# ducha-aiki/affnet

Measured on NVIDIA H100. Metric: Mpix/s end-to-end HesAffNet(+OriNet)+HardNet, higher is better.
Workload: dtype fp16 operands (fp16 residual planes: AffNet/OriNet weights+activations, HardNet layer 2-3 weights), fp32 accumulate; stencils fp32

## Files before the change

### affnet_b200/_lib.py

```python
import ctypes as C
import os
import subprocess

import torch

HERE = os.path.dirname(os.path.abspath(__file__))
LIB_PATH = os.environ.get("AFFNET_B200_LIB", os.path.join(HERE, "lib", "libaffnet_b200.so"))
AG_MAX_OCTAVES, AG_MAX_LEVELS = 16, 8
NET_AFFNET, NET_ORINET, NET_HARDNET = 0, 1, 2
ENGINE_SIMT, ENGINE_TC, ENGINE_TC_EXACT, ENGINE_TC_FAST, ENGINE_TC2, ENGINE_TC2_BF16 = 0, 1, 2, 3, 4, 5


class AffnetB200Error(RuntimeError):
    pass


class PyramidPlan(C.Structure):
    _fields_ = [
        ("B", C.c_int), ("H", C.c_int), ("W", C.c_int), ("n_octaves", C.c_int), ("n_levels", C.c_int),
        ("h", C.c_int * AG_MAX_OCTAVES), ("w", C.c_int * AG_MAX_OCTAVES),
        ("level_offset", (C.c_longlong * AG_MAX_LEVELS) * AG_MAX_OCTAVES),
        ("total_floats", C.c_longlong),
        ("sigma", (C.c_double * AG_MAX_LEVELS) * AG_MAX_OCTAVES),
        ("blur_sigma", (C.c_double * AG_MAX_LEVELS) * AG_MAX_OCTAVES),
        ("pix_dist", C.c_double * AG_MAX_OCTAVES),
    ]


class DetectWs(C.Structure):
    _fields_ = [
        ("B", C.c_int), ("cand_cap", C.c_int), ("n_level_slots", C.c_int),
        ("d_cand_val", C.c_void_p), ("d_cand_seq", C.c_void_p), ("d_cand_scyx", C.c_void_p), ("d_cand_aux", C.c_void_p),
        ("d_cand_count", C.c_void_p), ("d_level_pos", C.c_void_p), ("d_level_emit", C.c_void_p), ("d_variants", C.c_void_p),
        ("d_octave_maps", C.c_void_p),
    ]


class PipelineConfig(C.Structure):
    _fields_ = [
        ("B", C.c_int), ("H", C.c_int), ("W", C.c_int), ("num_features", C.c_int), ("nlevels", C.c_int),
        ("border", C.c_int), ("init_sigma", C.c_double), ("mrSize", C.c_double), ("do_ori", C.c_int),
        ("cand_cap", C.c_int),
    ]


SHAPE_NONE, SHAPE_AFFNET, SHAPE_BAUMBERG = 0, 1, 2
ORI_NONE, ORI_ORINET, ORI_HISTOGRAM = 0, 1, 2


class PipelineEstimators(C.Structure):
    _fields_ = [("shape", C.c_int), ("num_baum_iters", C.c_int), ("shape_ps", C.c_int), ("ori", C.c_int), ("ori_ps", C.c_int)]


DESC_HARDNET, DESC_SIFT = 0, 1


class PipelineDescriptor(C.Structure):
    _fields_ = [("kind", C.c_int), ("ps", C.c_int), ("clipval", C.c_float)]


vp, i32, f32, f64, sz = C.c_void_p, C.c_int, C.c_float, C.c_double, C.c_size_t
PROTOTYPES = {
    "ag_last_error": (C.c_char_p, []),
    "ag_abi_version": (i32, []),
    "ag_prof_begin": (i32, [vp]),
    "ag_prof_end": (i32, []),
    "ag_prof_get": (i32, [i32, C.POINTER(C.c_char_p), C.POINTER(f32)]),
    "ag_pyramid_plan": (i32, [i32, i32, i32, i32, f64, i32, C.POINTER(PyramidPlan)]),
    "ag_pyramid_build": (i32, [C.POINTER(PyramidPlan), vp, vp, vp]),
    "ag_gaussian_blur": (i32, [vp, vp, i32, i32, i32, f64, vp]),
    "ag_hessian_response": (i32, [vp, vp, i32, i32, i32, f64, f32, vp]),
    "ag_detect_ws_bytes": (sz, [C.POINTER(PyramidPlan), i32]),
    "ag_detect_ws_carve": (i32, [C.POINTER(PyramidPlan), i32, vp, C.POINTER(DetectWs)]),
    "ag_detect": (i32, [C.POINTER(PyramidPlan), vp, f32, i32, C.POINTER(DetectWs), vp]),
    "ag_detect_level_from_responses": (i32, [vp, vp, vp, i32, i32, C.POINTER(f64), i32, vp, vp, i32, C.POINTER(DetectWs), vp]),
    "ag_select_keypoints": (i32, [C.POINTER(PyramidPlan), C.POINTER(DetectWs), i32, f32, i32, vp, vp, vp, vp, vp, vp]),
    "ag_select_all_workspace_bytes": (sz, [C.POINTER(PyramidPlan), i32]),
    "ag_select_all_keypoints": (i32, [C.POINTER(PyramidPlan), C.POINTER(DetectWs), f32, i32, vp, sz, vp, vp, vp, vp, vp, vp]),
    "ag_extract_patches": (i32, [vp, i32, i32, i32, i32, vp, i32, i32, vp, vp]),
    "ag_extract_patches_pyr": (i32, [C.POINTER(PyramidPlan), vp, vp, vp, vp, vp, i32, i32, vp, vp]),
    "ag_pyramid_level_for_lafs": (i32, [C.POINTER(PyramidPlan), vp, i32, i32, vp, vp, vp]),
    "ag_net_create": (i32, [i32, vp, sz, C.POINTER(vp)]),
    "ag_net_destroy": (None, [vp]),
    "ag_net_blob_floats": (sz, [i32]),
    "ag_net_set_engine": (i32, [vp, i32]),
    "ag_net_get_engine": (i32, [vp]),
    "ag_net_workspace_bytes": (sz, [i32, i32]),
    "ag_mat2_compose": (i32, [vp, vp, vp, i32, vp]),
    "ag_lafs_left_multiply": (i32, [vp, vp, vp, i32, vp]),
    "ag_affnet_forward_raw": (i32, [vp, vp, i32, vp, vp, sz, vp]),
    "ag_orinet_forward_raw": (i32, [vp, vp, i32, vp, vp, sz, vp]),
    "ag_debug_pyramid_mode": (i32, [i32]),
    "ag_debug_tcx_layer": (i32, [vp, vp, i32, i32, vp, vp, sz, vp]),
    "ag_debug_libm": (i32, [vp, vp, i32, vp, vp, vp, vp]),
    "ag_debug_orientation_hist_pyr": (i32, [C.POINTER(PyramidPlan), vp, vp, vp, vp, vp, i32, i32, vp, vp, vp]),
    "ag_debug_baumberg_pyr": (i32, [C.POINTER(PyramidPlan), vp, vp, vp, vp, vp, i32, i32, i32, vp, vp, vp]),
    "ag_affnet_forward": (i32, [vp, vp, i32, vp, i32, vp, vp, sz, vp]),
    "ag_orinet_forward": (i32, [vp, vp, i32, vp, i32, vp, vp, vp, sz, vp]),
    "ag_hardnet_forward": (i32, [vp, vp, i32, vp, i32, vp, vp, sz, vp]),
    "ag_net_forward_pyr": (i32, [vp, C.POINTER(PyramidPlan), vp, vp, vp, vp, vp, i32, vp, vp, sz, vp]),
    "ag_affine_shape_filter": (i32, [vp, vp, vp, vp, vp, vp, i32, i32, i32, i32, vp, vp, vp, vp, vp, vp]),
    "ag_affine_shape_filter_all": (i32, [vp, vp, vp, vp, vp, vp, i32, i32, vp, vp, vp, vp, vp, vp]),
    "ag_lafs_apply_rotation": (i32, [vp, vp, i32, vp]),
    "ag_lafs_scale": (i32, [vp, vp, i32, f32, f32, f32, vp]),
    "ag_lafs_to_ell": (i32, [vp, i32, vp, vp]),
    "ag_circular_gauss_kernel": (i32, [i32, f64, vp]),
    "ag_orientation_hist": (i32, [vp, i32, i32, vp, vp, vp]),
    "ag_baumberg_shape": (i32, [vp, i32, i32, vp, vp, vp]),
    "ag_sift_windows": (i32, [i32, vp, vp, C.POINTER(i32), C.POINTER(i32)]),
    "ag_sift_describe": (i32, [vp, i32, i32, f32, vp, vp]),
    "ag_sift_describe_pyr": (i32, [C.POINTER(PyramidPlan), vp, vp, vp, vp, vp, i32, i32, f32, vp, vp]),
    "ag_distance_matrix": (i32, [vp, i32, vp, i32, i32, vp, vp]),
    "ag_match_snn_workspace_bytes": (sz, [i32, i32]),
    "ag_match_snn": (i32, [vp, i32, vp, i32, i32, f32, vp, sz, vp, vp, vp, vp, vp]),
    "ag_match_pairs_workspace_bytes": (sz, [i32, i32, i32, i32, i32]),
    "ag_match_pairs": (i32, [vp, vp, i32, i32, vp, vp, i32, i32, i32, vp, i32, f32, vp, sz, vp, vp, vp, vp, vp, vp, vp]),
    "ag_homography_ransac": (i32, [vp, i32, i32, vp, i32, i32, vp, i32, vp, vp, i32, f32, f32, i32, C.c_uint64, vp, vp, vp, vp, vp]),
    "ag_gt_correspondences_pairs": (i32, [vp, i32, i32, vp, i32, i32, vp, i32, vp, vp, i32, vp, f32, vp, vp, vp, vp, vp]),
    "ag_pipeline_create": (i32, [C.POINTER(PipelineConfig), vp, vp, vp, C.POINTER(vp)]),
    "ag_pipeline_create_ex": (i32, [C.POINTER(PipelineConfig), C.POINTER(PipelineEstimators), vp, vp, vp, C.POINTER(vp)]),
    "ag_pipeline_create_desc": (i32, [C.POINTER(PipelineConfig), C.POINTER(PipelineEstimators), C.POINTER(PipelineDescriptor), vp, vp, vp,
                                      C.POINTER(vp)]),
    "ag_pipeline_create_th": (i32, [C.POINTER(PipelineConfig), C.POINTER(PipelineEstimators), C.POINTER(PipelineDescriptor), f32, vp, vp, vp,
                                    C.POINTER(vp)]),
    "ag_pipeline_destroy": (None, [vp]),
    "ag_pipeline_workspace_bytes": (sz, [vp]),
    "ag_pipeline_plan": (C.POINTER(PyramidPlan), [vp]),
    "ag_pipeline_run": (i32, [vp, vp, vp, sz, vp, vp, vp, vp, vp]),
    "ag_pipeline_launch_count": (i32, [vp]),
}

_lib = None


def build(verbose=False):
    r = subprocess.run(["bash", os.path.join(HERE, "csrc", "build.sh")], capture_output=True, text=True)
    if r.returncode != 0:
        raise AffnetB200Error("building libaffnet_b200.so failed:\n" + r.stdout + r.stderr)
    if verbose:
        print(r.stdout.strip())
    return LIB_PATH


def lib():
    global _lib
    if _lib is None:
        if not os.path.isfile(LIB_PATH):
            raise AffnetB200Error("%s not found: run `python -c 'import __graft_entry__ as g; g.build()'` "
                                  "(there is no CPU fallback)" % LIB_PATH)
        L = C.CDLL(LIB_PATH)
        for name, (res, args) in PROTOTYPES.items():
            fn = getattr(L, name)
            fn.restype, fn.argtypes = res, args
        _lib = L
    return _lib


def check(rc):
    if rc != 0:
        raise AffnetB200Error("libaffnet_b200 error %d: %s" % (rc, lib().ag_last_error().decode()))


def stream_ptr():
    return C.c_void_p(torch.cuda.current_stream().cuda_stream)


def ptr(t):
    if t is None:
        return C.c_void_p(0)
    return C.c_void_p(t.data_ptr())


def require_cuda(t, name="tensor"):
    if not (isinstance(t, torch.Tensor) and t.is_cuda):
        raise AffnetB200Error("%s must be a CUDA tensor: affnet_b200 has no CPU path" % name)
    return t


def f32c(t, name="tensor"):
    require_cuda(t, name)
    if t.dtype != torch.float32:
        t = t.float()
    return t.contiguous()


def make_plan(B, H, W, nlevels=3, init_sigma=1.6, border=5):
    plan = PyramidPlan()
    check(lib().ag_pyramid_plan(B, H, W, nlevels, float(init_sigma), border, C.byref(plan)))
    return plan


def profile(fn):
    check(lib().ag_prof_begin(stream_ptr()))
    try:
        fn()
    finally:
        n = lib().ag_prof_end()
    if n < 0:
        check(n)
    out = []
    for i in range(n):
        name, ms = C.c_char_p(), C.c_float()
        check(lib().ag_prof_get(i, C.byref(name), C.byref(ms)))
        out.append((name.value.decode(), ms.value))
    return out
```

### affnet_b200/csrc/net_impl.cuh

```cuda
#pragma once
#include <cuda_fp16.h>

#include <vector>

#include "common.cuh"

#define AG_ENGINE_SIMT 0
#define AG_ENGINE_TC 1
#define AG_ENGINE_TC_EXACT 2
#define AG_ENGINE_TC2 4
#define AG_ENGINE_TC2_BF16 5
#define AG_ENGINE_TC_FAST 3

struct ag_net {
    int kind;
    int engine;
    float* d_w[6];
    float* d_b[6];
    float* d_w1;
    __half* d_wx[6];
    __half* d_all_x;
    __half* d_wx_bf[6];
    __half* d_headh_bf;
    __half* d_wh[6];
    __half* d_headh;
    float* d_head_w;
    float* d_head_b;
    float* d_head_bx;
    float w_inv_scale[6];
    float head_inv_scale;
    float* d_all;
    __half* d_all_h;
};

#include "tc_conv.cuh"

namespace ag {
size_t tc_act_bytes(int kind);
int tc_nsplit(int kind, int layer);
int tc_split_w(int kind);
tc::FirstSrc tc_src_patches(const float* patches);
tc::FirstSrc tc_src_pyramid(const ag_pyramid_plan_t* p, const float* pyr, const float* lafs, const int* oct, const int* lvl, int cap);
int tc_hardnet_forward(const ag_net* net, const tc::FirstSrc& src, int n, int group, const int* count, void* bufA, void* bufB, void* headbuf,
                       float* out, cudaStream_t st);
int tc_trunk_orinet(const ag_net* net, const tc::FirstSrc& src, int n, int group, const int* count, void* bufA, void* bufB, void* feat,
                    cudaStream_t st);
int tc_trunk_affnet(const ag_net* net, const tc::FirstSrc& src, int n, int group, const int* count, void* bufA, void* bufB, void* feat,
                    cudaStream_t st);
int tc_headx_forward(const ag_net* net, const void* feat, int n, int group, const int* count, float* out, float* angle, cudaStream_t st, float* raw = nullptr);
size_t tc_headx_bytes(int n);
void tcx_pack_layer(const float* wf, int ci, int co, int stride, int nsplit, int sw, float scale, std::vector<__half>& out, int bf16 = 0);
int tcx_nsplit(int kind, int layer);
int tcx_split_w(int kind, int layer);
int tcx_stride(int layer);
size_t tcx_act_bytes(int n);
int tcx_trunk_affori(const ag_net* net, const tc::FirstSrc& src, int n, int group, const int* count, void* bufA, void* bufB, void* feat,
                     cudaStream_t st, int upto);
int tcx_trunk_hardnet(const ag_net* net, const tc::FirstSrc& src, int n, int group, const int* count, void* bufA, void* bufB, void* headbuf,
                      cudaStream_t st, int upto, int bf16 = 0);
int tc_hardnet_head(const ag_net* net, const void* headbuf, int n, int group, const int* count, float* out, cudaStream_t st, int bf16 = 0);
}
```

### affnet_b200/csrc/nets_simt.cu

```cuda
#include <math.h>

#include <vector>

#include <cuda_bf16.h>

#include "net_impl.cuh"

namespace ag {

constexpr float BN_EPS = 1e-5f;
constexpr int CNT = 256;

struct LayerCfg {
    int cin, cout, stride, hin;
};
static const LayerCfg kAffCfg[6] = {{1, 16, 1, 32}, {16, 16, 1, 32}, {16, 32, 2, 32}, {32, 32, 1, 16}, {32, 64, 2, 16}, {64, 64, 1, 8}};
static const LayerCfg kHardCfg[6] = {{1, 32, 1, 32}, {32, 32, 1, 32}, {32, 64, 2, 32}, {64, 64, 1, 16}, {64, 128, 2, 16}, {128, 128, 1, 8}};

}

namespace ag {

template <int CIN, int COUT, int HIN, int STRIDE, int CT, int CK, bool NORM>
__global__ void __launch_bounds__(CNT) conv3x3_kernel(const float* __restrict__ in, float* __restrict__ out,
                                                       const float* __restrict__ wpk, const float* __restrict__ bias,
                                                       int group, const int* __restrict__ count) {
    constexpr int HOUT = HIN / STRIDE, NP = HOUT * HOUT, PPT = 4, PT = NP / PPT, CGN = CNT / PT, CPT = CT / CGN;
    constexpr int HP = HIN + 2, WP = HIN + 2;
    static_assert(PT * CGN == CNT && CPT * CGN == CT && CPT % 4 == 0, "bad tiling");
    static_assert(CIN % CK == 0, "bad cin chunk");
    extern __shared__ float smem[];
    float* s_in = smem;
    float* s_w = smem + CIN * HP * WP;
    __shared__ float s_red[CNT / 32][2];

    const int pi = blockIdx.x;
    if (count != nullptr && (pi % group) >= count[pi / group]) return;
    const int ct0 = blockIdx.y * CT;
    const float* src = in + (size_t)pi * CIN * HIN * HIN;

    float mean = 0.f, inv = 1.f;
    if (NORM) {
        float s = 0.f;
        for (int i = threadIdx.x; i < HIN * HIN; i += CNT) s += src[i];
        for (int o = 16; o > 0; o >>= 1) s += __shfl_xor_sync(0xffffffffu, s, o);
        if ((threadIdx.x & 31) == 0) s_red[threadIdx.x >> 5][0] = s;
        __syncthreads();
        s = 0.f;
        for (int i = 0; i < CNT / 32; i++) s += s_red[i][0];
        mean = s / (float)(HIN * HIN);
        float q = 0.f;
        for (int i = threadIdx.x; i < HIN * HIN; i += CNT) { const float d = src[i] - mean; q = fmaf(d, d, q); }
        for (int o = 16; o > 0; o >>= 1) q += __shfl_xor_sync(0xffffffffu, q, o);
        if ((threadIdx.x & 31) == 0) s_red[threadIdx.x >> 5][1] = q;
        __syncthreads();
        q = 0.f;
        for (int i = 0; i < CNT / 32; i++) q += s_red[i][1];
        inv = 1.f / (sqrtf(q / (float)(HIN * HIN - 1)) + 1e-7f);
    }
    for (int i = threadIdx.x; i < CIN * HP * WP; i += CNT) {
        const int c = i / (HP * WP), r = i - c * HP * WP, y = r / WP, x = r - y * WP;
        float v = 0.f;
        if (y >= 1 && y <= HIN && x >= 1 && x <= HIN) {
            v = src[(size_t)c * HIN * HIN + (y - 1) * HIN + (x - 1)];
            if (NORM) v = (v - mean) * inv;
        }
        s_in[i] = v;
    }

    const int pt = threadIdx.x % PT, cg = threadIdx.x / PT;
    int poff[PPT];
#pragma unroll
    for (int k = 0; k < PPT; k++) {
        const int p = pt + k * PT, y = p / HOUT, x = p - y * HOUT;
        poff[k] = (y * STRIDE) * WP + x * STRIDE;
    }
    float acc[PPT][CPT];
#pragma unroll
    for (int j = 0; j < CPT; j++) {
        const float bv = bias[ct0 + cg * CPT + j];
#pragma unroll
        for (int k = 0; k < PPT; k++) acc[k][j] = bv;
    }

    for (int c0 = 0; c0 < CIN; c0 += CK) {
        __syncthreads();
        for (int i = threadIdx.x; i < 9 * CK * CT; i += CNT) {
            const int tap = i / (CK * CT), r = i - tap * CK * CT, c = r / CT, co = r - c * CT;
            s_w[i] = __ldg(wpk + ((size_t)tap * CIN + c0 + c) * COUT + ct0 + co);
        }
        __syncthreads();
#pragma unroll 1
        for (int c = 0; c < CK; c++) {
            const float* ip = s_in + (c0 + c) * HP * WP;
#pragma unroll
            for (int tap = 0; tap < 9; tap++) {
                const int toff = (tap / 3) * WP + (tap % 3);
                float a[PPT];
#pragma unroll
                for (int k = 0; k < PPT; k++) a[k] = ip[poff[k] + toff];
                const float4* wp = reinterpret_cast<const float4*>(s_w + (tap * CK + c) * CT + cg * CPT);
#pragma unroll
                for (int j4 = 0; j4 < CPT / 4; j4++) {
                    const float4 wv = wp[j4];
#pragma unroll
                    for (int k = 0; k < PPT; k++) {
                        acc[k][j4 * 4 + 0] = fmaf(a[k], wv.x, acc[k][j4 * 4 + 0]);
                        acc[k][j4 * 4 + 1] = fmaf(a[k], wv.y, acc[k][j4 * 4 + 1]);
                        acc[k][j4 * 4 + 2] = fmaf(a[k], wv.z, acc[k][j4 * 4 + 2]);
                        acc[k][j4 * 4 + 3] = fmaf(a[k], wv.w, acc[k][j4 * 4 + 3]);
                    }
                }
            }
        }
    }
    float* dst = out + (size_t)pi * COUT * NP;
#pragma unroll
    for (int j = 0; j < CPT; j++)
#pragma unroll
        for (int k = 0; k < PPT; k++) dst[(size_t)(ct0 + cg * CPT + j) * NP + pt + k * PT] = fmaxf(acc[k][j], 0.f);
}

template <int CIN, int COUT, int HIN, int STRIDE, int CT, int CK, bool NORM>
static int launch_conv(const float* in, float* out, const float* w, const float* b, int n, int group, const int* count,
                       cudaStream_t st) {
    constexpr size_t smem = sizeof(float) * ((size_t)CIN * (HIN + 2) * (HIN + 2) + 9 * CK * CT);
    static SmemAttrOnce attr_once;
    auto kern = conv3x3_kernel<CIN, COUT, HIN, STRIDE, CT, CK, NORM>;
    {
        int rc = attr_once.ensure(kern, smem, "conv smem attr");
        if (rc != AG_OK) return rc;
    }
    kern<<<dim3(n, COUT / CT), CNT, smem, st>>>(in, out, w, b, group, count);
    AG_CHECK_LAUNCH("conv3x3_kernel");
    return AG_OK;
}

__device__ __forceinline__ float warp_sum(float v) {
    for (int o = 16; o > 0; o >>= 1) v += __shfl_xor_sync(0xffffffffu, v, o);
    return v;
}

__global__ void affnet_head_kernel(const float* __restrict__ feat, const float* __restrict__ w, const float* __restrict__ bias,
                                   float* __restrict__ out, int n, int group, const int* __restrict__ count) {
    const int pi = blockIdx.x * (blockDim.x >> 5) + (threadIdx.x >> 5), lane = threadIdx.x & 31;
    if (pi >= n) return;
    if (count != nullptr && (pi % group) >= count[pi / group]) return;
    const float* f = feat + (size_t)pi * 4096;
    float s0 = 0.f, s1 = 0.f, s2 = 0.f;
    for (int i = lane; i < 4096; i += 32) {
        const float v = f[i];
        s0 = fmaf(v, __ldg(w + i), s0); s1 = fmaf(v, __ldg(w + 4096 + i), s1); s2 = fmaf(v, __ldg(w + 8192 + i), s2);
    }
    s0 = warp_sum(s0); s1 = warp_sum(s1); s2 = warp_sum(s2);
    if (lane == 0) {
        const float a00 = 1.0f + tanhf(s0 + bias[0]), a10 = tanhf(s1 + bias[1]), a11 = 1.0f + tanhf(s2 + bias[2]);
        rectify_up_is_up(a00, 0.f, a10, a11, out + (size_t)pi * 4);
    }
}

constexpr int OH_P = 4, OH_W = 8, OH_KC = 256;
__global__ void __launch_bounds__(OH_W * 32) orinet_head_kernel(const float* __restrict__ feat, const float* __restrict__ weff, const float* __restrict__ bias,
                                                                 float* __restrict__ out, float* __restrict__ angle_out, int n, int group,
                                                                 const int* __restrict__ count) {
    __shared__ __align__(16) float s_w[OH_KC][20];
    const int warp = threadIdx.x >> 5, lane = threadIdx.x & 31;
    const int p0 = (blockIdx.x * OH_W + warp) * OH_P;
    float acc[OH_P][18];
#pragma unroll
    for (int q = 0; q < OH_P; q++)
#pragma unroll
        for (int o = 0; o < 18; o++) acc[q][o] = 0.f;
    const float* f[OH_P];
#pragma unroll
    for (int q = 0; q < OH_P; q++) f[q] = feat + (size_t)min(p0 + q, n - 1) * 4096;
    for (int k0 = 0; k0 < 4096; k0 += OH_KC) {
        __syncthreads();
        for (int i = threadIdx.x; i < OH_KC * 18; i += OH_W * 32) s_w[i / 18][i % 18] = __ldg(weff + (size_t)k0 * 18 + i);
        __syncthreads();
#pragma unroll 2
        for (int kk = lane; kk < OH_KC; kk += 32) {
            float v[OH_P];
#pragma unroll
            for (int q = 0; q < OH_P; q++) v[q] = f[q][k0 + kk];
            const float4* wr = reinterpret_cast<const float4*>(&s_w[kk][0]);
            const float4 w0 = wr[0], w1 = wr[1], w2 = wr[2], w3 = wr[3];
            const float2 w4 = *reinterpret_cast<const float2*>(&s_w[kk][16]);
            const float wv[18] = {w0.x, w0.y, w0.z, w0.w, w1.x, w1.y, w1.z, w1.w, w2.x, w2.y, w2.z, w2.w, w3.x, w3.y, w3.z, w3.w, w4.x, w4.y};
#pragma unroll
            for (int q = 0; q < OH_P; q++)
#pragma unroll
                for (int o = 0; o < 18; o++) acc[q][o] = fmaf(v[q], wv[o], acc[q][o]);
        }
    }
#pragma unroll
    for (int q = 0; q < OH_P; q++) {
        float m0 = 0.f, m1 = 0.f;
#pragma unroll
        for (int o = 0; o < 9; o++) {
            m0 += tanhf(warp_sum(acc[q][o]) + bias[0]);
            m1 += tanhf(warp_sum(acc[q][9 + o]) + bias[1]);
        }
        const int pi = p0 + q;
        if (lane != 0 || pi >= n) continue;
        if (count != nullptr && (pi % group) >= count[pi / group]) continue;
        m0 /= 9.0f; m1 /= 9.0f;
        const float ang = atan2f(m0 + 1e-8f, m1 + 1e-8f);
        if (angle_out) angle_out[pi] = ang;
        if (out) {
            const float c = cosf(ang), sn = sinf(ang);
            float* o = out + (size_t)pi * 4;
            o[0] = c; o[1] = sn; o[2] = -sn; o[3] = c;
        }
    }
}

constexpr int HH_P = 16;
__global__ void __launch_bounds__(256) hardnet_head_kernel(const float* __restrict__ feat, const float* __restrict__ w,
                                                            const float* __restrict__ bn, float* __restrict__ out, int n,
                                                            int group, const int* __restrict__ count) {
    __shared__ float s_a[HH_P][64 + 1];
    const int p0 = blockIdx.x * HH_P;
    const int co = threadIdx.x & 127, half = threadIdx.x >> 7;
    float acc[HH_P / 2];
#pragma unroll
    for (int k = 0; k < HH_P / 2; k++) acc[k] = 0.f;
    for (int k0 = 0; k0 < 8192; k0 += 64) {
        __syncthreads();
        for (int i = threadIdx.x; i < HH_P * 64; i += 256) {
            const int p = i >> 6, k = i & 63;
            s_a[p][k] = (p0 + p < n) ? feat[(size_t)(p0 + p) * 8192 + k0 + k] : 0.f;
        }
        __syncthreads();
#pragma unroll 8
        for (int k = 0; k < 64; k++) {
            const float wv = __ldg(w + (size_t)(k0 + k) * 128 + co);
#pragma unroll
            for (int q = 0; q < HH_P / 2; q++) acc[q] = fmaf(s_a[half * (HH_P / 2) + q][k], wv, acc[q]);
        }
    }
    const float sc = bn[co], sh = bn[128 + co];
    float v[HH_P / 2];
#pragma unroll
    for (int q = 0; q < HH_P / 2; q++) v[q] = fmaf(acc[q], sc, sh);
    __syncthreads();
    const int wih = (threadIdx.x >> 5) & 3;
#pragma unroll
    for (int q = 0; q < HH_P / 2; q++) {
        const float ss = warp_sum(v[q] * v[q]);
        if ((threadIdx.x & 31) == 0) s_a[half * (HH_P / 2) + q][wih] = ss;
    }
    __syncthreads();
#pragma unroll
    for (int q = 0; q < HH_P / 2; q++) {
        const int r = half * (HH_P / 2) + q, p = p0 + r;
        if (p >= n) continue;
        if (count != nullptr && (p % group) >= count[p / group]) continue;
        const float ss = (s_a[r][0] + s_a[r][1]) + (s_a[r][2] + s_a[r][3]);
        out[(size_t)p * 128 + co] = v[q] / sqrtf(ss + 1e-8f);
    }
}

static float pow2_scale(const float* w, size_t n) {
    float wmax = 0.f;
    for (size_t i = 0; i < n; i++) wmax = fmaxf(wmax, fabsf(w[i]));
    int ex = 0;
    if (wmax > 0.f) { frexpf(wmax, &ex); ex = 13 - ex; }
    return ldexpf(1.0f, ex);
}

static size_t blob_floats(int kind) {
    const LayerCfg* cfg = (kind == AG_NET_HARDNET) ? kHardCfg : kAffCfg;
    size_t n = 0;
    for (int l = 0; l < 6; l++) n += (size_t)cfg[l].cout * cfg[l].cin * 9 + 2 * cfg[l].cout;
    const int c = cfg[5].cout;
    if (kind == AG_NET_HARDNET) n += (size_t)128 * c * 64 + 256;
    else n += (size_t)(kind == AG_NET_AFFNET ? 3 : 2) * c * 64 + (kind == AG_NET_AFFNET ? 3 : 2);
    return n;
}

}

using namespace ag;

extern "C" {

size_t ag_net_blob_floats(int kind) {
    if (kind < 0 || kind > 2) return 0;
    return blob_floats(kind);
}

int ag_net_create(int kind, const float* h_blob, size_t n_floats, ag_net_t** out) {
    AG_REQUIRE(out && h_blob, "NULL argument");
    AG_REQUIRE(kind >= 0 && kind <= 2, "unknown net kind");
    if (n_floats != blob_floats(kind)) {
        set_error("ag_net_create: blob has %zu floats, kind %d needs %zu", n_floats, kind, blob_floats(kind));
        return AG_ERR_INVALID;
    }
    const LayerCfg* cfg = (kind == AG_NET_HARDNET) ? kHardCfg : kAffCfg;
    std::vector<float> packed;
    size_t w_off[6], b_off[6], hw_off, hb_off;
    const float* p = h_blob;
    for (int l = 0; l < 6; l++) {
        const int ci = cfg[l].cin, co = cfg[l].cout;
        const float* w = p; const float* mean = w + (size_t)co * ci * 9; const float* var = mean + co;
        p = var + co;
        w_off[l] = packed.size();
        packed.resize(packed.size() + (size_t)9 * ci * co);
        float* dst = packed.data() + w_off[l];
        std::vector<float> invstd(co);
        for (int o = 0; o < co; o++) invstd[o] = 1.0f / sqrtf(var[o] + BN_EPS);
        for (int tap = 0; tap < 9; tap++)
            for (int c = 0; c < ci; c++)
                for (int o = 0; o < co; o++) dst[((size_t)tap * ci + c) * co + o] = w[((size_t)o * ci + c) * 9 + tap] * invstd[o];
        while (packed.size() % 4) packed.push_back(0.f);
        b_off[l] = packed.size();
        for (int o = 0; o < co; o++) packed.push_back(-mean[o] * invstd[o]);
        while (packed.size() % 4) packed.push_back(0.f);
    }
    const int c = cfg[5].cout;
    hw_off = packed.size();
    if (kind == AG_NET_HARDNET) {
        const float* w = p; const float* mean = w + (size_t)128 * c * 64; const float* var = mean + 128;
        packed.resize(packed.size() + (size_t)8192 * 128);
        float* dst = packed.data() + hw_off;
        for (int o = 0; o < 128; o++)
            for (int k = 0; k < 8192; k++) dst[(size_t)k * 128 + o] = w[(size_t)o * 8192 + k];
        hb_off = packed.size();
        for (int o = 0; o < 128; o++) packed.push_back(1.0f / sqrtf(var[o] + BN_EPS));
        for (int o = 0; o < 128; o++) packed.push_back(-mean[o] / sqrtf(var[o] + BN_EPS));
    } else {
        const int no = (kind == AG_NET_AFFNET) ? 3 : 2;
        const float* w = p; const float* bias = w + (size_t)no * c * 64;
        if (kind == AG_NET_ORINET) {
            packed.resize(packed.size() + (size_t)4096 * 18);
            float* dst = packed.data() + hw_off;
            for (int ci = 0; ci < 64; ci++)
                for (int y = 0; y < 8; y++)
                    for (int x = 0; x < 8; x++)
                        for (int ch = 0; ch < 2; ch++)
                            for (int oy = 0; oy < 3; oy++)
                                for (int ox = 0; ox < 3; ox++) {
                                    const int ky = y - oy + 1, kx = x - ox + 1;
                                    const float v = (ky >= 0 && ky < 8 && kx >= 0 && kx < 8) ? w[((size_t)ch * 64 + ci) * 64 + ky * 8 + kx] : 0.f;
                                    dst[((size_t)ci * 64 + y * 8 + x) * 18 + ch * 9 + oy * 3 + ox] = v;
                                }
        } else
            packed.insert(packed.end(), w, w + (size_t)no * c * 64);
        hb_off = packed.size();
        packed.insert(packed.end(), bias, bias + no);
        while (packed.size() % 4) packed.push_back(0.f);
    }
    std::vector<__half> packed_h;
    size_t wh_off[6] = {0, 0, 0, 0, 0, 0};
    float w_scale[6] = {1.f, 1.f, 1.f, 1.f, 1.f, 1.f};
    w_scale[0] = pow2_scale(packed.data() + w_off[0], (size_t)9 * cfg[0].cout);
    const int sw = tc_split_w(kind);
    for (int l = 1; l < 6; l++) {
        const int ci = cfg[l].cin, co = cfg[l].cout, ns = tc_nsplit(kind, l), nt = co / ns, kc = ci / 8;
        const float* wf = packed.data() + w_off[l];
        w_scale[l] = pow2_scale(wf, (size_t)9 * ci * co);
        wh_off[l] = packed_h.size();
        packed_h.resize(packed_h.size() + (size_t)9 * ci * co * (1 + sw));
        __half* dst = packed_h.data() + wh_off[l];
        for (int sp = 0; sp < ns; sp++)
            for (int tap = 0; tap < 9; tap++)
                for (int g = 0; g < kc; g++)
                    for (int part = 0; part <= sw; part++)
                        for (int nn = 0; nn < nt; nn++)
                            for (int e = 0; e < 8; e++) {
                                const float v = w_scale[l] * wf[((size_t)tap * ci + g * 8 + e) * co + sp * nt + nn];
                                const __half hi = __float2half_rn(v);
                                const __half val = part == 0 ? hi : __float2half_rn(v - __half2float(hi));
                                dst[(((((size_t)sp * 9 + tap) * kc + g) * (1 + sw) + part) * nt + nn) * 8 + e] = val;
                            }
    }
    std::vector<__half> packed_x;
    size_t wx_off[6] = {0, 0, 0, 0, 0, 0};
    for (int l = 1; l < 6; l++) {
        wx_off[l] = packed_x.size();
        tcx_pack_layer(packed.data() + w_off[l], cfg[l].cin, cfg[l].cout, tcx_stride(l), tcx_nsplit(kind, l), tcx_split_w(kind, l), w_scale[l], packed_x);
        while (packed_x.size() % 8) packed_x.push_back(__float2half_rn(0.f));
    }
    std::vector<__half> packed_bf;
    size_t wbf_off[6] = {0, 0, 0, 0, 0, 0}, headbf_off = 0;
    if (kind == AG_NET_HARDNET) {
        for (int l = 1; l < 6; l++) {
            wbf_off[l] = packed_bf.size();
            tcx_pack_layer(packed.data() + w_off[l], cfg[l].cin, cfg[l].cout, tcx_stride(l), tcx_nsplit(kind, l), tcx_split_w(kind, l), w_scale[l], packed_bf, 1);
            while (packed_bf.size() % 8) packed_bf.push_back(__float2half_rn(0.f));
        }
        headbf_off = packed_bf.size();
        packed_bf.resize(packed_bf.size() + (size_t)8192 * 128);
        const float* hw = packed.data() + hw_off;
        for (int pix = 0; pix < 64; pix++)
            for (int cg = 0; cg < 16; cg++)
                for (int o = 0; o < 128; o++)
                    for (int e = 0; e < 8; e++) {
                        const __nv_bfloat16 bv = __float2bfloat16_rn(hw[((size_t)(cg * 8 + e) * 64 + pix) * 128 + o]);
                        memcpy(&packed_bf[headbf_off + (((size_t)(pix * 16 + cg)) * 128 + o) * 8 + e], &bv, 2);
                    }
    }
    size_t headh_off = 0, hbx_off = 0;
    float head_scale = 1.0f;
    if (kind == AG_NET_HARDNET) {
        while (packed_h.size() % 8) packed_h.push_back(__float2half_rn(0.f));
        headh_off = packed_h.size();
        packed_h.resize(packed_h.size() + (size_t)8192 * 128);
        __half* dst = packed_h.data() + headh_off;
        const float* hw = packed.data() + hw_off;
        const float hs = pow2_scale(hw, (size_t)8192 * 128);
        for (int pix = 0; pix < 64; pix++)
            for (int cg = 0; cg < 16; cg++)
                for (int o = 0; o < 128; o++)
                    for (int e = 0; e < 8; e++)
                        dst[(((size_t)(pix * 16 + cg)) * 128 + o) * 8 + e] = __float2half_rn(hs * hw[((size_t)(cg * 8 + e) * 64 + pix) * 128 + o]);
        hbx_off = packed.size();
        for (int o = 0; o < 128; o++) packed.push_back(packed[hb_off + o] * (1.0f / hs));
        for (int o = 0; o < 128; o++) packed.push_back(packed[hb_off + 128 + o]);
    }
    if (kind != AG_NET_HARDNET) {
        const int no = (kind == AG_NET_AFFNET) ? 3 : 18;
        while (packed_h.size() % 8) packed_h.push_back(__float2half_rn(0.f));
        headh_off = packed_h.size();
        packed_h.resize(packed_h.size() + (size_t)4096 * 64, __float2half_rn(0.f));
        __half* dst = packed_h.data() + headh_off;
        const float* hw = packed.data() + hw_off;
        head_scale = pow2_scale(hw, (size_t)4096 * no);
        for (int pix = 0; pix < 64; pix++)
            for (int cg = 0; cg < 8; cg++)
                for (int o = 0; o < no; o++)
                    for (int e = 0; e < 8; e++) {
                        const size_t k = (size_t)(cg * 8 + e) * 64 + pix;
                        const float v = head_scale * ((kind == AG_NET_AFFNET) ? hw[(size_t)o * 4096 + k] : hw[k * 18 + o]);
                        const __half hi = __float2half_rn(v);
                        const size_t chunk = (size_t)pix * 8 + cg;
                        dst[(chunk * 64 + o) * 8 + e] = hi;
                        dst[(chunk * 64 + 32 + o) * 8 + e] = __float2half_rn(v - __half2float(hi));
                    }
    }
    ag_net* net = new ag_net();
    memset(net, 0, sizeof(*net));
    net->kind = kind;
    net->engine = AG_ENGINE_TC2;
    net->head_inv_scale = 1.0f / head_scale;
    for (int l = 0; l < 6; l++) net->w_inv_scale[l] = 1.0f / w_scale[l];
    {
        int rch = check_cuda(cudaMalloc(&net->d_all_h, packed_h.size() * sizeof(__half)), "cudaMalloc fp16 weights");
        if (rch != AG_OK) { delete net; return rch; }
        rch = check_cuda(cudaMemcpy(net->d_all_h, packed_h.data(), packed_h.size() * sizeof(__half), cudaMemcpyHostToDevice), "upload fp16 weights");
        if (rch != AG_OK) { cudaFree(net->d_all_h); delete net; return rch; }
        for (int l = 1; l < 6; l++) net->d_wh[l] = net->d_all_h + wh_off[l];
        net->d_headh = net->d_all_h + headh_off;
        rch = check_cuda(cudaMalloc(&net->d_all_x, packed_x.size() * sizeof(__half)), "cudaMalloc fp16 weights (second generation)");
        if (rch == AG_OK) rch = check_cuda(cudaMemcpy(net->d_all_x, packed_x.data(), packed_x.size() * sizeof(__half), cudaMemcpyHostToDevice), "upload fp16 weights");
        if (rch != AG_OK) { cudaFree(net->d_all_h); cudaFree(net->d_all_x); delete net; return rch; }
        for (int l = 1; l < 6; l++) net->d_wx[l] = net->d_all_x + wx_off[l];
        if (!packed_bf.empty()) {
            __half* dbf = nullptr;
            rch = check_cuda(cudaMalloc(&dbf, packed_bf.size() * sizeof(__half)), "cudaMalloc bf16 weights");
            if (rch == AG_OK) rch = check_cuda(cudaMemcpy(dbf, packed_bf.data(), packed_bf.size() * sizeof(__half), cudaMemcpyHostToDevice), "upload bf16 weights");
            if (rch != AG_OK) { cudaFree(dbf); cudaFree(net->d_all_h); cudaFree(net->d_all_x); delete net; return rch; }
            net->d_wx_bf[0] = dbf;
            for (int l = 1; l < 6; l++) net->d_wx_bf[l] = dbf + wbf_off[l];
            net->d_headh_bf = dbf + headbf_off;
        }
    }
    int rc = check_cuda(cudaMalloc(&net->d_all, packed.size() * sizeof(float)), "cudaMalloc weights");
    if (rc != AG_OK) { cudaFree(net->d_all_h); cudaFree(net->d_all_x); delete net; return rc; }
    rc = check_cuda(cudaMemcpy(net->d_all, packed.data(), packed.size() * sizeof(float), cudaMemcpyHostToDevice), "upload weights");
    if (rc != AG_OK) { cudaFree(net->d_all); cudaFree(net->d_all_h); cudaFree(net->d_all_x); delete net; return rc; }
    for (int l = 0; l < 6; l++) { net->d_w[l] = net->d_all + w_off[l]; net->d_b[l] = net->d_all + b_off[l]; }
    net->d_w1 = net->d_w[0];
    net->d_head_w = net->d_all + hw_off;
    net->d_head_b = net->d_all + hb_off;
    net->d_head_bx = net->d_all + hbx_off;
    *out = net;
    return AG_OK;
}

void ag_net_destroy(ag_net_t* net) {
    if (!net) return;
    cudaFree(net->d_all);
    cudaFree(net->d_all_h);
    cudaFree(net->d_all_x);
    cudaFree(net->d_wx_bf[0]);
    delete net;
}

int ag_net_set_engine(ag_net_t* net, int engine) {
    AG_REQUIRE(net != nullptr, "NULL net");
    AG_REQUIRE(engine == AG_ENGINE_SIMT || engine == AG_ENGINE_TC || engine == AG_ENGINE_TC_EXACT || engine == AG_ENGINE_TC_FAST || engine == AG_ENGINE_TC2 || engine == AG_ENGINE_TC2_BF16, "unknown engine");
    AG_REQUIRE(engine != AG_ENGINE_TC2_BF16 || net->kind == AG_NET_HARDNET, "the bf16 engine exists for HardNet only");
    AG_REQUIRE(engine != AG_ENGINE_TC_FAST || net->kind == AG_NET_AFFNET, "the fast tensor-core engine exists for AffNet only");
    AG_REQUIRE(engine != AG_ENGINE_TC_EXACT || net->kind != AG_NET_HARDNET, "the exact tensor-core engine exists for AffNet / OriNet");
    net->engine = engine;
    return AG_OK;
}

int ag_net_get_engine(const ag_net_t* net) { return net ? net->engine : -1; }

size_t ag_net_workspace_bytes(int kind, int n) {
    if (n <= 0) return 0;
    const size_t per = (kind == AG_NET_HARDNET) ? 32768 : 16384;
    const size_t simt = 2 * align_up((size_t)n * per * sizeof(float), 256);
    const size_t act1 = (size_t)n * tc_act_bytes(kind == AG_NET_AFFNET ? AG_NET_ORINET : kind), act2 = tcx_act_bytes(n);
    const size_t tcb = 2 * align_up(act1 > act2 ? act1 : act2, 256) +
                       (kind == AG_NET_HARDNET ? align_up(((size_t)n + 128) * 8192 * 2, 256) : align_up(tc_headx_bytes(n), 256));
    return simt > tcb ? simt : tcb;
}

}

namespace ag {

static int trunk_affnet(const ag_net* net, const float* patches, int n, int group, const int* count, float* a, float* b,
                        cudaStream_t st) {
    int rc;
    if ((rc = launch_conv<1, 16, 32, 1, 16, 1, true>(patches, a, net->d_w[0], net->d_b[0], n, group, count, st))) return rc;
    if ((rc = launch_conv<16, 16, 32, 1, 16, 16, false>(a, b, net->d_w[1], net->d_b[1], n, group, count, st))) return rc;
    if ((rc = launch_conv<16, 32, 32, 2, 32, 16, false>(b, a, net->d_w[2], net->d_b[2], n, group, count, st))) return rc;
    if ((rc = launch_conv<32, 32, 16, 1, 32, 32, false>(a, b, net->d_w[3], net->d_b[3], n, group, count, st))) return rc;
    if ((rc = launch_conv<32, 64, 16, 2, 64, 32, false>(b, a, net->d_w[4], net->d_b[4], n, group, count, st))) return rc;
    if ((rc = launch_conv<64, 64, 8, 1, 64, 32, false>(a, b, net->d_w[5], net->d_b[5], n, group, count, st))) return rc;
    return AG_OK;
}

static int trunk_hardnet(const ag_net* net, const float* patches, int n, int group, const int* count, float* a, float* b,
                         cudaStream_t st) {
    int rc;
    if ((rc = launch_conv<1, 32, 32, 1, 32, 1, true>(patches, a, net->d_w[0], net->d_b[0], n, group, count, st))) return rc;
    if ((rc = launch_conv<32, 32, 32, 1, 32, 32, false>(a, b, net->d_w[1], net->d_b[1], n, group, count, st))) return rc;
    if ((rc = launch_conv<32, 64, 32, 2, 64, 32, false>(b, a, net->d_w[2], net->d_b[2], n, group, count, st))) return rc;
    if ((rc = launch_conv<64, 64, 16, 1, 64, 32, false>(a, b, net->d_w[3], net->d_b[3], n, group, count, st))) return rc;
    if ((rc = launch_conv<64, 128, 16, 2, 128, 16, false>(b, a, net->d_w[4], net->d_b[4], n, group, count, st))) return rc;
    if ((rc = launch_conv<128, 128, 8, 1, 128, 16, false>(a, b, net->d_w[5], net->d_b[5], n, group, count, st))) return rc;
    return AG_OK;
}

static int run_trunk(const ag_net* net, const float* patches, const tc::FirstSrc* pyr_src, int n, int group, const int* count, float* a,
                     float* b, float** feat, cudaStream_t st) {
    if (net->engine != AG_ENGINE_SIMT) {
        const tc::FirstSrc src = pyr_src ? *pyr_src : tc_src_patches(patches);
        char* base = (char*)a;
        const size_t total = 2 * (size_t)((char*)b - (char*)a);
        const size_t act = net->engine == AG_ENGINE_TC2 ? align_up(tcx_act_bytes(n), 256)
                                                        : align_up((size_t)n * tc_act_bytes(net->engine == AG_ENGINE_TC_FAST ? net->kind : AG_NET_ORINET), 256);
        const size_t fbytes = tc_headx_bytes(n);
        if (2 * act + fbytes > total) { set_error("tensor-core workspace too small"); return AG_ERR_CAPACITY; }
        void* bufA = base;
        void* bufB = base + act;
        b = (float*)(base + 2 * act);
        *feat = b;
        if (net->kind == AG_NET_HARDNET) { set_error("HardNet tensor-core path has its own entry"); return AG_ERR_INVALID; }
        if (net->engine == AG_ENGINE_TC2) return tcx_trunk_affori(net, src, n, group, count, bufA, bufB, b, st, 6);
        if (net->engine != AG_ENGINE_TC_FAST) return tc_trunk_orinet(net, src, n, group, count, bufA, bufB, b, st);
        return tc_trunk_affnet(net, src, n, group, count, bufA, bufB, b, st);
    }
    *feat = b;
    if (patches == nullptr) { set_error("the fp32 SIMT engine needs materialised patches"); return AG_ERR_INVALID; }
    return net->kind == AG_NET_HARDNET ? trunk_hardnet(net, patches, n, group, count, a, b, st)
                                       : trunk_affnet(net, patches, n, group, count, a, b, st);
}

static int split_ws(int kind, int n, void* d_ws, size_t ws_bytes, float** a, float** b) {
    const size_t need = ag_net_workspace_bytes(kind, n);
    if (d_ws == nullptr || ws_bytes < need) {
        set_error("net forward: workspace of %zu bytes needed, %zu given", need, ws_bytes);
        return AG_ERR_CAPACITY;
    }
    *a = (float*)d_ws;
    *b = (float*)((char*)d_ws + need / 2);
    return AG_OK;
}

}

extern "C" {

static int affnet_impl(const ag_net_t* net, const float* d_patches, const tc::FirstSrc* src, int n, const int* d_count, int group,
                       float* d_out, void* d_ws, size_t ws_bytes, void* stream, float* d_raw = nullptr) {
    AG_REQUIRE(net && (d_patches || src) && (d_out || d_raw), "NULL argument");
    AG_REQUIRE(net->kind == AG_NET_AFFNET, "not an AffNet handle");
    if (n <= 0) return AG_OK;
    if (group <= 0) group = n;
    float *a, *b;
    int rc = split_ws(net->kind, n, d_ws, ws_bytes, &a, &b);
    if (rc) return rc;
    cudaStream_t st = (cudaStream_t)stream;
    if ((rc = run_trunk(net, d_patches, src, n, group, d_count, a, b, &b, st))) return rc;
    if (net->engine == AG_ENGINE_TC || net->engine == AG_ENGINE_TC_FAST || net->engine == AG_ENGINE_TC2) return tc_headx_forward(net, b, n, group, d_count, d_out, nullptr, st, d_raw);
    AG_REQUIRE(d_raw == nullptr && d_out, "raw head outputs need a tensor-core engine with the GEMM head (1, 3 or 4)");
    affnet_head_kernel<<<cdiv(n, 8), 256, 0, st>>>(b, net->d_head_w, net->d_head_b, d_out, n, group, d_count);
    AG_CHECK_LAUNCH("affnet_head_kernel");
    return AG_OK;
}

static int orinet_impl(const ag_net_t* net, const float* d_patches, const tc::FirstSrc* src, int n, const int* d_count, int group,
                       float* d_out, float* d_angle, void* d_ws, size_t ws_bytes, void* stream, float* d_raw = nullptr) {
    AG_REQUIRE(net && (d_patches || src) && (d_out || d_angle || d_raw), "NULL argument");
    AG_REQUIRE(net->kind == AG_NET_ORINET, "not an OriNet handle");
    if (n <= 0) return AG_OK;
    if (group <= 0) group = n;
    float *a, *b;
    int rc = split_ws(net->kind, n, d_ws, ws_bytes, &a, &b);
    if (rc) return rc;
    cudaStream_t st = (cudaStream_t)stream;
    if ((rc = run_trunk(net, d_patches, src, n, group, d_count, a, b, &b, st))) return rc;
    if (net->engine == AG_ENGINE_TC || net->engine == AG_ENGINE_TC2) return tc_headx_forward(net, b, n, group, d_count, d_out, d_angle, st, d_raw);
    AG_REQUIRE(d_raw == nullptr, "raw head outputs need a tensor-core engine with the GEMM head (1 or 4)");
    orinet_head_kernel<<<cdiv(n, OH_W * OH_P), OH_W * 32, 0, st>>>(b, net->d_head_w, net->d_head_b, d_out, d_angle, n, group, d_count);
    AG_CHECK_LAUNCH("orinet_head_kernel");
    return AG_OK;
}

static int hardnet_impl(const ag_net_t* net, const float* d_patches, const tc::FirstSrc* src, int n, const int* d_count, int group,
                        float* d_out, void* d_ws, size_t ws_bytes, void* stream) {
    AG_REQUIRE(net && (d_patches || src) && d_out, "NULL argument");
    AG_REQUIRE(net->kind == AG_NET_HARDNET, "not a HardNet handle");
    if (n <= 0) return AG_OK;
    if (group <= 0) group = n;
    float *a, *b;
    int rc = split_ws(net->kind, n, d_ws, ws_bytes, &a, &b);
    if (rc) return rc;
    cudaStream_t st = (cudaStream_t)stream;
    if (net->engine == AG_ENGINE_TC2 || net->engine == AG_ENGINE_TC2_BF16) {
        const int bf = net->engine == AG_ENGINE_TC2_BF16;
        char* base = (char*)d_ws;
        const size_t act = align_up(tcx_act_bytes(n), 256);
        const tc::FirstSrc s0 = src ? *src : tc_src_patches(d_patches);
        if ((rc = tcx_trunk_hardnet(net, s0, n, group, d_count, base, base + act, base + 2 * act, st, 6, bf))) return rc;
        return tc_hardnet_head(net, base + 2 * act, n, group, d_count, d_out, st, bf);
    }
    if (net->engine == AG_ENGINE_TC) {
        char* base = (char*)d_ws;
        const size_t act = align_up((size_t)n * tc_act_bytes(net->kind), 256);
        const tc::FirstSrc s0 = src ? *src : tc_src_patches(d_patches);
        return tc_hardnet_forward(net, s0, n, group, d_count, base, base + act, base + 2 * act, d_out, st);
    }
    if ((rc = run_trunk(net, d_patches, src, n, group, d_count, a, b, &b, st))) return rc;
    hardnet_head_kernel<<<cdiv(n, HH_P), 256, 0, st>>>(b, net->d_head_w, net->d_head_b, d_out, n, group, d_count);
    AG_CHECK_LAUNCH("hardnet_head_kernel");
    return AG_OK;
}

int ag_affnet_forward(const ag_net_t* net, const float* d_patches, int n, const int* d_count, int group, float* d_out, void* d_ws,
                      size_t ws_bytes, void* stream) {
    AG_REQUIRE(d_patches, "NULL patches");
    return affnet_impl(net, d_patches, nullptr, n, d_count, group, d_out, d_ws, ws_bytes, stream);
}
int ag_orinet_forward(const ag_net_t* net, const float* d_patches, int n, const int* d_count, int group, float* d_out, float* d_angle,
                      void* d_ws, size_t ws_bytes, void* stream) {
    AG_REQUIRE(d_patches, "NULL patches");
    return orinet_impl(net, d_patches, nullptr, n, d_count, group, d_out, d_angle, d_ws, ws_bytes, stream);
}
int ag_affnet_forward_raw(const ag_net_t* net, const float* d_patches, int n, float* d_raw, void* d_ws, size_t ws_bytes, void* stream) {
    AG_REQUIRE(d_patches && d_raw, "NULL argument");
    return affnet_impl(net, d_patches, nullptr, n, nullptr, n, nullptr, d_ws, ws_bytes, stream, d_raw);
}
int ag_orinet_forward_raw(const ag_net_t* net, const float* d_patches, int n, float* d_raw, void* d_ws, size_t ws_bytes, void* stream) {
    AG_REQUIRE(d_patches && d_raw, "NULL argument");
    return orinet_impl(net, d_patches, nullptr, n, nullptr, n, nullptr, nullptr, d_ws, ws_bytes, stream, d_raw);
}
int ag_hardnet_forward(const ag_net_t* net, const float* d_patches, int n, const int* d_count, int group, float* d_out, void* d_ws,
                       size_t ws_bytes, void* stream) {
    AG_REQUIRE(d_patches, "NULL patches");
    return hardnet_impl(net, d_patches, nullptr, n, d_count, group, d_out, d_ws, ws_bytes, stream);
}

int ag_net_forward_pyr(const ag_net_t* net, const ag_pyramid_plan_t* plan, const float* d_pyr, const float* d_lafs, const int* d_oct,
                       const int* d_lvl, const int* d_count, int cap, float* d_out, void* d_ws, size_t ws_bytes, void* stream) {
    AG_REQUIRE(net && plan && d_pyr && d_lafs && d_oct && d_lvl && d_out, "NULL argument");
    AG_REQUIRE(cap >= 1, "bad capacity");
    AG_REQUIRE(net->engine != AG_ENGINE_SIMT, "fused sampling needs a tensor-core engine");
    const tc::FirstSrc src = tc_src_pyramid(plan, d_pyr, d_lafs, d_oct, d_lvl, cap);
    const int n = plan->B * cap;
    if (net->kind == AG_NET_AFFNET) return affnet_impl(net, nullptr, &src, n, d_count, cap, d_out, d_ws, ws_bytes, stream);
    if (net->kind == AG_NET_ORINET) return orinet_impl(net, nullptr, &src, n, d_count, cap, d_out, nullptr, d_ws, ws_bytes, stream);
    return hardnet_impl(net, nullptr, &src, n, d_count, cap, d_out, d_ws, ws_bytes, stream);
}

}
```

### affnet_b200/csrc/nets_tcx.cu

```cuda
#include <stdlib.h>
#include <string.h>

#include <vector>

#include <cuda_bf16.h>

#include "net_impl.cuh"
#include "tcx_conv.cuh"
#include "tcx_first.cuh"

namespace ag {
namespace tcx {

static int num_sms() {
    static int n = 0;
    if (n == 0) {
        int dev = 0;
        cudaGetDevice(&dev);
        cudaDeviceGetAttribute(&n, cudaDevAttrMultiProcessorCount, dev);
        if (n <= 0) n = 132;
    }
    return n;
}

static int ensure_smem_attr(const void* func, int bytes, bool* configured, const char* what) {
    int dev = 0;
    cudaGetDevice(&dev);
    dev &= 63;
    if (configured[dev]) return AG_OK;
    int rc = check_cuda(cudaFuncSetAttribute(func, cudaFuncAttributeMaxDynamicSharedMemorySize, bytes), what);
    if (rc == AG_OK) configured[dev] = true;
    return rc;
}

template <int CIN, int COUT, int H, int STRIDE, int NSPLIT, int STAGES, int OUT, int SA, int SW, int OSA, int BF = 0, int MC = 0, int PPS = 0>
static int launch_conv(const void* in, void* out, const __half* w, const float* b, float inv_scale, int n, int group, const int* count, cudaStream_t st) {
    using Cfg = XCfg<CIN, COUT, H, STRIDE, NSPLIT, STAGES, OUT, SA, SW, OSA>;
    auto kern = tcx_conv_kernel<CIN, COUT, H, STRIDE, NSPLIT, STAGES, OUT, SA, SW, OSA, BF, MC, PPS>;
    static bool configured[64] = {};
    int rc = ensure_smem_attr((const void*)kern, (int)Cfg::SMEM, configured, "tcx_conv smem attr");
    if (rc != AG_OK) return rc;
    XArgs a;
    a.in = (const __half*)in; a.out = out; a.wpk = w; a.bias = b; a.inv_scale = inv_scale; a.n = n; a.group = group; a.count = count;
    const int units = Cfg::In::PAIR ? (n + 1) / 2 : n;
    int gx = num_sms() / NSPLIT;
    if (gx > units) gx = units;
    if (gx < 1) gx = 1;
    if (MC) {
        cudaLaunchConfig_t cfg;
        memset(&cfg, 0, sizeof(cfg));
        cfg.gridDim = dim3(gx, NSPLIT); cfg.blockDim = dim3(Cfg::THREADS); cfg.dynamicSmemBytes = Cfg::SMEM; cfg.stream = st;
        cudaLaunchAttribute attr[1];
        attr[0].id = cudaLaunchAttributeClusterDimension;
        attr[0].val.clusterDim.x = 1; attr[0].val.clusterDim.y = 2; attr[0].val.clusterDim.z = 1;
        cfg.attrs = attr; cfg.numAttrs = 1;
        rc = check_cuda(cudaLaunchKernelEx(&cfg, kern, a), "tcx_conv cluster launch");
        if (rc != AG_OK) return rc;
    } else
        kern<<<dim3(gx, NSPLIT), Cfg::THREADS, Cfg::SMEM, st>>>(a);
    AG_CHECK_LAUNCH("tcx_conv_kernel");
    return AG_OK;
}

template <int C1, int COUT, int SA, int SW, int OSA, int BF = 0, int L3 = 0>
static int launch_first(void* out, const __half* w, const float* b, float inv_scale, int n, int group, const int* count, cudaStream_t st, const FirstSrc& src,
                        void* out3 = nullptr, const __half* w3 = nullptr, const float* b3 = nullptr, float inv_scale3 = 0.f) {
    using Cfg = XFirstCfg<C1, COUT, SA, SW, OSA, L3>;
    auto kern = tcx_first_kernel<C1, COUT, SA, SW, OSA, BF, L3>;
    static bool configured[64] = {};
    int rc = ensure_smem_attr((const void*)kern, (int)Cfg::SMEM, configured, "tcx_first smem attr");
    if (rc != AG_OK) return rc;
    XArgs a;
    a.in = nullptr; a.out = out; a.wpk = w; a.bias = b; a.inv_scale = inv_scale; a.n = n; a.group = group; a.count = count;
    XArgs a3 = a;
    a3.out = out3; a3.wpk = w3; a3.bias = b3; a3.inv_scale = inv_scale3;
    int gx = num_sms();
    if (gx > n) gx = n;
    if (gx < 1) gx = 1;
    kern<<<gx, Cfg::THREADS, Cfg::SMEM, st>>>(a, src, a3);
    AG_CHECK_LAUNCH("tcx_first_kernel");
    return AG_OK;
}

__global__ void tcx_decode_kernel(const __half* __restrict__ buf, int layout, int C, int osa, int H, int n, int bf, float* __restrict__ out) {
    const size_t total = (size_t)n * C * H * H;
    auto val = [&](size_t k) -> float { return bf ? __uint_as_float((uint32_t)__half_as_ushort(buf[k]) << 16) : __half2float(buf[k]); };
    for (size_t i = (size_t)blockIdx.x * blockDim.x + threadIdx.x; i < total; i += (size_t)gridDim.x * blockDim.x) {
        const int x = (int)(i % H), y = (int)((i / H) % H), c = (int)((i / ((size_t)H * H)) % C), pi = (int)(i / ((size_t)H * H * C));
        size_t hi, lo;
        if (layout == L_HEAD) {
            const size_t tile = (size_t)H * H * (C / 8) * 128 * 8;
            hi = (size_t)(pi >> 7) * tile + ((((size_t)(y * H + x) * (C / 8) + c / 8) * 128 + (pi & 127)) * 8 + (c & 7));
            lo = hi + (size_t)((n + 127) >> 7) * tile;
        } else {
            const int slots = layout_slots(layout);
            const size_t unit_halfs = (size_t)(C / 8) * slots * 8 * (osa ? 2 : 1);
            const int unit = layout_pair(layout) ? (pi >> 1) : pi;
            const int slot = layout_slot(layout, y, x, pi & 1);
            hi = (size_t)unit * unit_halfs + ((size_t)(c / 8) * slots + slot) * 8 + (c & 7);
            lo = hi + (size_t)(C / 8) * slots * 8;
        }
        float v = val(hi);
        if (osa) v += val(lo);
        out[i] = v;
    }
}

}

static __half bf16_bits_as_half(float v) {
    const __nv_bfloat16 b = __float2bfloat16_rn(v);
    __half h;
    memcpy(&h, &b, 2);
    return h;
}
static float bf16_round(float v) { return __bfloat162float(__float2bfloat16_rn(v)); }

void tcx_pack_layer(const float* wf, int ci, int co, int stride, int nsplit, int sw, float scale, std::vector<__half>& out, int bf16) {
    const int nt = co / nsplit;
    auto put = [&](int dy, int dx, int cin, int c, int part) {
        const float v = scale * wf[((size_t)(dy * 3 + dx) * ci + cin) * co + c];
        if (bf16) {
            const float hi = bf16_round(v);
            out.push_back(bf16_bits_as_half(part == 0 ? hi : v - hi));
        } else {
            const __half hi = __float2half_rn(v);
            out.push_back(part == 0 ? hi : __float2half_rn(v - __half2float(hi)));
        }
    };
    for (int sp = 0; sp < nsplit; sp++)
        for (int dy = 0; dy < 3; dy++)
            for (int j = 0; j < ci / 16; j++) {
                if (stride == 1) {
                    for (int kg = 0; kg < 2; kg++)
                        for (int part = 0; part <= sw; part++)
                            for (int dx = 0; dx < 3; dx++)
                                for (int c = 0; c < nt; c++)
                                    for (int e = 0; e < 8; e++) put(dy, dx, (2 * j + kg) * 8 + e, sp * nt + c, part);
                } else {
                    for (int kg = 0; kg < 2; kg++)
                        for (int part = 0; part <= sw; part++)
                            for (int dx = 0; dx < 3; dx += 2)
                                for (int c = 0; c < nt; c++)
                                    for (int e = 0; e < 8; e++) put(dy, dx, (2 * j + kg) * 8 + e, sp * nt + c, part);
                    for (int kg = 0; kg < 2; kg++)
                        for (int part = 0; part <= sw; part++)
                            for (int c = 0; c < nt; c++)
                                for (int e = 0; e < 8; e++) put(dy, 1, (2 * j + kg) * 8 + e, sp * nt + c, part);
                }
            }
}

int tcx_nsplit(int kind, int layer) { return (kind == AG_NET_HARDNET && layer >= 4) ? 2 : 1; }
#ifndef AG_HARD_SW2
#define AG_HARD_SW2 1
#endif
#ifndef AG_HARD_SW3
#define AG_HARD_SW3 1
#endif
#ifndef AG_HARD_SW4
#define AG_HARD_SW4 0
#endif
int tcx_split_w(int kind, int layer) { return kind == AG_NET_HARDNET ? (layer == 1 ? AG_HARD_SW2 : layer == 2 ? AG_HARD_SW3 : layer == 3 ? AG_HARD_SW4 : 0) : 1; }
int tcx_stride(int layer) { return (layer == 2 || layer == 4) ? 2 : 1; }

size_t tcx_act_bytes(int n) { return (size_t)(n + 1) * 65536; }

#ifndef AG_HARD_MC5
#define AG_HARD_MC5 1
#endif
#ifndef AG_HARD_MC6
#define AG_HARD_MC6 0
#endif
int tcx_trunk_affori(const ag_net* net, const tc::FirstSrc& src0, int n, int group, const int* count, void* bufA, void* bufB, void* feat,
                     cudaStream_t st, int upto) {
    using namespace tcx;
    tc::FirstSrc src = src0;
    src.w1 = net->d_w1; src.b1 = net->d_b[0]; src.w1_inv = net->w_inv_scale[0]; src.w1_scale = 1.0f / net->w_inv_scale[0];
    int rc;
    if (upto <= 2) return launch_first<16, 16, 1, 1, 1>(bufB, net->d_wx[1], net->d_b[1], net->w_inv_scale[1], n, group, count, st, src);
    if ((rc = launch_first<16, 16, 1, 1, 1, 0, 1>(nullptr, net->d_wx[1], net->d_b[1], net->w_inv_scale[1], n, group, count, st, src,
                                                   bufA, net->d_wx[2], net->d_b[2], net->w_inv_scale[2]))) return rc;
    if (upto <= 3) return AG_OK;
    if ((rc = launch_conv<32, 32, 16, 1, 1, 4, L_S2_8P, 1, 1, 1>(bufA, bufB, net->d_wx[3], net->d_b[3], net->w_inv_scale[3], n, group, count, st))) return rc;
    if (upto <= 4) return AG_OK;
    if ((rc = launch_conv<32, 64, 16, 2, 1, 2, L_S1_8P, 1, 1, 1>(bufB, bufA, net->d_wx[4], net->d_b[4], net->w_inv_scale[4], n, group, count, st))) return rc;
    if (upto <= 5) return AG_OK;
    return launch_conv<64, 64, 8, 1, 1, 2, L_HEAD, 1, 1, 1, 0, 0, 1>(bufA, feat, net->d_wx[5], net->d_b[5], net->w_inv_scale[5], n, group, count, st);
}

template <int BF>
static int trunk_hardnet_t(const ag_net* net, const tc::FirstSrc& src0, int n, int group, const int* count, void* bufA, void* bufB, void* headbuf,
                           cudaStream_t st, int upto) {
    using namespace tcx;
    tc::FirstSrc src = src0;
    src.w1 = net->d_w1; src.b1 = net->d_b[0]; src.w1_inv = net->w_inv_scale[0]; src.w1_scale = 1.0f / net->w_inv_scale[0];
    __half* const* wx = BF ? net->d_wx_bf : net->d_wx;
    int rc;
    if ((rc = launch_first<32, 32, 0, AG_HARD_SW2, 0, BF>(bufB, wx[1], net->d_b[1], net->w_inv_scale[1], n, group, count, st, src))) return rc;
    if (upto <= 2) return AG_OK;
    if ((rc = launch_conv<32, 64, 32, 2, 1, 2, L_S1_16, 0, AG_HARD_SW3, 0, BF>(bufB, bufA, wx[2], net->d_b[2], net->w_inv_scale[2], n, group, count, st))) return rc;
    if (upto <= 3) return AG_OK;
    if ((rc = launch_conv<64, 64, 16, 1, 1, 2, L_S2_8P, 0, AG_HARD_SW4, 0, BF>(bufA, bufB, wx[3], net->d_b[3], net->w_inv_scale[3], n, group, count, st))) return rc;
    if (upto <= 4) return AG_OK;
    if ((rc = launch_conv<64, 128, 16, 2, 2, 2, L_S1_8P, 0, 0, 0, BF, AG_HARD_MC5, 1>(bufB, bufA, wx[4], net->d_b[4], net->w_inv_scale[4], n, group, count, st))) return rc;
    if (upto <= 5) return AG_OK;
    return launch_conv<128, 128, 8, 1, 2, 2, L_HEAD, 0, 0, 0, BF, AG_HARD_MC6, 1>(bufA, headbuf, wx[5], net->d_b[5], net->w_inv_scale[5], n, group, count, st);
}

int tcx_trunk_hardnet(const ag_net* net, const tc::FirstSrc& src0, int n, int group, const int* count, void* bufA, void* bufB, void* headbuf,
                      cudaStream_t st, int upto, int bf16) {
    return bf16 ? trunk_hardnet_t<1>(net, src0, n, group, count, bufA, bufB, headbuf, st, upto)
                : trunk_hardnet_t<0>(net, src0, n, group, count, bufA, bufB, headbuf, st, upto);
}

}

using namespace ag;

extern "C" {

int ag_debug_tcx_layer(const ag_net_t* net, const float* d_patches, int n, int upto, float* d_out, void* d_ws, size_t ws_bytes, void* stream) {
    AG_REQUIRE(net && d_patches && d_out && d_ws, "NULL argument");
    AG_REQUIRE(upto >= 2 && upto <= 6 && n >= 1, "layer out of range");
    const size_t act = align_up(tcx_act_bytes(n), 256);
    AG_REQUIRE(ws_bytes >= ag_net_workspace_bytes(net->kind, n), "workspace too small");
    cudaStream_t st = (cudaStream_t)stream;
    char* base = (char*)d_ws;
    const tc::FirstSrc src = tc_src_patches(d_patches);
    const bool hard = net->kind == AG_NET_HARDNET;
    const int bf = hard && net->engine == AG_ENGINE_TC2_BF16;
    int rc = hard ? tcx_trunk_hardnet(net, src, n, n, nullptr, base, base + act, base + 2 * act, st, upto, bf)
                  : tcx_trunk_affori(net, src, n, n, nullptr, base, base + act, base + 2 * act, st, upto);
    if (rc) return rc;
    const int lay = upto == 2 ? tcx::L_S2_16 : upto == 3 ? tcx::L_S1_16 : upto == 4 ? tcx::L_S2_8P : upto == 5 ? tcx::L_S1_8P : tcx::L_HEAD;
    const int H = upto == 2 ? 32 : (upto <= 4 ? 16 : 8);
    const int Cb = hard ? 32 : 16;
    const int C = upto == 2 ? Cb : (upto <= 4 ? 2 * Cb : 4 * Cb);
    const void* buf = upto == 6 ? base + 2 * act : (upto == 2 || upto == 4) ? base + act : base;
    const int osa = hard ? 0 : 1;
    tcx::tcx_decode_kernel<<<296, 256, 0, st>>>((const __half*)buf, lay, C, osa, H, n, bf, d_out);
    AG_CHECK_LAUNCH("tcx_decode_kernel");
    return AG_OK;
}

#ifdef AG_FIRST_TIMELINE
int ag_first_timeline_read(unsigned long long* host, int* dims, int reset) {
    constexpr size_t n = (size_t)tcx::TL_LAUNCHES * tcx::TL_CTAS * 16 * tcx::TL_STATES;
    if (dims) { dims[0] = tcx::TL_LAUNCHES; dims[1] = tcx::TL_CTAS; dims[2] = tcx::TL_STATES; }
    cudaDeviceSynchronize();
    if (host) {
        const int rc = check_cuda(cudaMemcpyFromSymbol(host, tcx::g_first_tl, n * 8), "timeline read");
        if (rc != AG_OK) return rc;
    }
    if (reset) {
        static unsigned long long zeros[n];
        static int zl[tcx::TL_CTAS];
        int rc = check_cuda(cudaMemcpyToSymbol(tcx::g_first_tl, zeros, sizeof(zeros)), "timeline reset");
        if (rc == AG_OK) rc = check_cuda(cudaMemcpyToSymbol(tcx::g_first_tl_launch, zl, sizeof(zl)), "timeline reset");
        return rc;
    }
    return AG_OK;
}
#endif

#ifdef AG_CONV_TIMELINE
int ag_conv_timeline_read(unsigned long long* sums, unsigned long long* events, int* dims, int reset) {
    using namespace tcx;
    if (dims) { dims[0] = CT_LAUNCHES; dims[1] = CT_CTAS; dims[2] = CT_STATES; dims[3] = CT_EVENTS; }
    int rc = check_cuda(cudaDeviceSynchronize(), "timeline read");
    if (rc == AG_OK && sums) rc = check_cuda(cudaMemcpyFromSymbol(sums, g_conv_tl, sizeof(g_conv_tl)), "timeline read");
    if (rc == AG_OK && events) rc = check_cuda(cudaMemcpyFromSymbol(events, g_conv_ev, sizeof(g_conv_ev)), "timeline read");
    if (rc == AG_OK && reset) {
        void* p = nullptr;
        const int zl[CT_CTAS] = {};
        if (rc == AG_OK) rc = check_cuda(cudaGetSymbolAddress(&p, g_conv_tl), "timeline reset");
        if (rc == AG_OK) rc = check_cuda(cudaMemset(p, 0, sizeof(g_conv_tl)), "timeline reset");
        if (rc == AG_OK) rc = check_cuda(cudaGetSymbolAddress(&p, g_conv_ev), "timeline reset");
        if (rc == AG_OK) rc = check_cuda(cudaMemset(p, 0, sizeof(g_conv_ev)), "timeline reset");
        if (rc == AG_OK) rc = check_cuda(cudaMemcpyToSymbol(g_conv_tl_launch, zl, sizeof(zl)), "timeline reset");
        if (rc == AG_OK) rc = check_cuda(cudaDeviceSynchronize(), "timeline reset");
    }
    return rc;
}
#endif

}
```

### affnet_b200/csrc/tcx_conv.cuh

```cuda
#pragma once
#include <cuda_bf16.h>

#include "tc_conv.cuh"

#ifndef AG_CONV_PINGPONG
#define AG_CONV_PINGPONG 1
#endif

namespace ag {
namespace tcx {

using namespace ag::tc;

constexpr int XORDER = 5;

enum { CT_TOTAL, CT_WAIT_FULL, CT_TURN, CT_ISSUE, CT_MMA_WAIT, CT_EPILOGUE, CT_WG_BAR, CT_WAIT_EMPTY, CT_OTHER, CT_STATES };
#ifdef AG_CONV_TIMELINE
constexpr int CT_CTAS = 4, CT_LAUNCHES = 16, CT_EVENTS = 2048;
__device__ unsigned long long g_conv_tl[CT_LAUNCHES][CT_CTAS][9][CT_STATES];
__device__ unsigned long long g_conv_ev[CT_LAUNCHES][2][CT_EVENTS][3];
__device__ int g_conv_tl_launch[CT_CTAS];
struct ConvTimeline {
    unsigned long long t[CT_STATES];
    long long start, mark;
    int slot, warp, n_ev;
    __device__ static void claim(int* s_slot) {
        if (threadIdx.x == 0)
            *s_slot = (blockIdx.y == 0 && blockIdx.x < CT_CTAS) ? min(atomicAdd(&g_conv_tl_launch[blockIdx.x], 1), CT_LAUNCHES) : CT_LAUNCHES;
    }
    __device__ void init(const int* s_slot) {
        for (int i = 0; i < CT_STATES; i++) t[i] = 0;
        slot = *s_slot; warp = threadIdx.x >> 5; n_ev = 0;
        start = mark = clock64();
    }
    __device__ void lap(int state) { const long long now = clock64(); t[state] += (unsigned long long)(now - mark); mark = now; }
    __device__ void event(int k) {
        if (blockIdx.x == 0 && slot < CT_LAUNCHES && (threadIdx.x & 127) == 0 && n_ev < CT_EVENTS) g_conv_ev[slot][warp >> 2][n_ev][k] = (unsigned long long)mark;
        if (k == 2) n_ev++;
    }
    __device__ void finish() {
        t[CT_TOTAL] = (unsigned long long)(clock64() - start);
        if ((threadIdx.x & 31) == 0 && slot < CT_LAUNCHES)
            for (int i = 0; i < CT_STATES; i++) g_conv_tl[slot][blockIdx.x][warp][i] = t[i];
    }
};
#else
struct ConvTimeline {
    __device__ static void claim(int*) {}
    __device__ void init(const int*) {}
    __device__ void lap(int) {}
    __device__ void event(int) {}
    __device__ void finish() {}
};
#endif

enum XLayout { L_S2_16 = 0, L_S1_16 = 1, L_S2_8P = 2, L_S1_8P = 3, L_HEAD = 4 };

__device__ __forceinline__ void bulk_g2s_mc(void* dst, const void* src, uint32_t bytes, uint64_t* bar, uint16_t mask) {
    asm volatile("cp.async.bulk.shared::cluster.global.mbarrier::complete_tx::bytes.multicast::cluster [%0], [%1], %2, [%3], %4;" ::"r"(smem_u32(dst)),
                 "l"(src), "r"(bytes), "r"(smem_u32(bar)), "h"(mask)
                 : "memory");
}
__device__ __forceinline__ void mbar_arrive_cluster(uint64_t* bar, uint32_t cta) {
    asm volatile("{\n .reg .b32 ra;\n mapa.shared::cluster.u32 ra, %0, %1;\n mbarrier.arrive.release.cta.shared::cluster.b64 _, [ra];\n}\n" ::"r"(smem_u32(bar)), "r"(cta)
                 : "memory");
}
__device__ __forceinline__ void cluster_sync() {
    asm volatile("barrier.cluster.arrive.release.aligned;\n barrier.cluster.wait.acquire.aligned;" ::: "memory");
}

template <int BF>
__device__ __forceinline__ uint32_t pack2(float a, float b) {
    if (BF) { const __nv_bfloat162 h = __floats2bfloat162_rn(a, b); return *reinterpret_cast<const uint32_t*>(&h); }
    const __half2 h = __floats2half2_rn(a, b);
    return *reinterpret_cast<const uint32_t*>(&h);
}
template <int BF>
__device__ __forceinline__ float2 unpack2(uint32_t u) {
    if (BF) return make_float2(__uint_as_float(u << 16), __uint_as_float(u & 0xFFFF0000u));
    return __half22float2(*reinterpret_cast<const __half2*>(&u));
}
template <int LO, int BF = 0>
__device__ __forceinline__ void split_pack8(const float* v, uint4& hi, uint4& lo) {
    uint32_t h[4], l[4];
#pragma unroll
    for (int i = 0; i < 4; i++) {
        h[i] = pack2<BF>(v[2 * i], v[2 * i + 1]);
        if (LO) {
            const float2 f = unpack2<BF>(h[i]);
            l[i] = pack2<BF>(v[2 * i] - f.x, v[2 * i + 1] - f.y);
        } else l[i] = 0;
    }
    hi = make_uint4(h[0], h[1], h[2], h[3]);
    lo = make_uint4(l[0], l[1], l[2], l[3]);
}

template <int LO, int BF = 0>
__device__ __forceinline__ void split_pack2(float v0, float v1, uint32_t& hi, uint32_t& lo) {
    hi = pack2<BF>(v0, v1);
    if (LO) {
        const float2 f = unpack2<BF>(hi);
        lo = pack2<BF>(v0 - f.x, v1 - f.y);
    } else lo = 0;
}

__host__ __device__ constexpr int layout_slots(int lay) { return lay == L_S2_16 ? 1024 : lay == L_S1_16 ? 256 : lay == L_S2_8P ? 512 : 128; }
__host__ __device__ constexpr int layout_pair(int lay) { return (lay == L_S2_8P || lay == L_S1_8P) ? 1 : 0; }
__host__ __device__ constexpr int rpos(int x) { return (x & 1) * 8 + (x >> 1); }
__host__ __device__ constexpr int ppos(int x, int p) { return (x & 1) * 8 + p * 4 + (x >> 1); }
__host__ __device__ constexpr int layout_slot(int lay, int y, int x, int p) {
    return lay == L_S2_16 ? ((y & 1) * 2 + (x & 1)) * 256 + (y >> 1) * 16 + rpos(x >> 1)
         : lay == L_S1_16 ? y * 16 + rpos(x)
         : lay == L_S2_8P ? ((y & 1) * 2 + (x & 1)) * 128 + (y >> 1) * 16 + ppos(x >> 1, p)
                          : y * 16 + ppos(x, p);
}

template <int H, int STRIDE>
struct XIn {
    static constexpr int HOUT = H / STRIDE;
    static constexpr int PAIR = (HOUT == 8) ? 1 : 0;
    static constexpr int W = HOUT;
    static constexpr int RW = W * (1 + PAIR);
    static constexpr int TILES = HOUT * RW / 128;
    static constexpr int NPLANES = (STRIDE == 1) ? 1 : 4;
    static constexpr int DATA = HOUT * RW;
    static constexpr int PLANE = DATA + RW;
    static constexpr int SLOT_STAGE = NPLANES * PLANE;
    static constexpr int LAYOUT = (STRIDE == 2) ? (PAIR ? L_S2_8P : L_S2_16) : (PAIR ? L_S1_8P : L_S1_16);
    static_assert(HOUT == 8 || HOUT == 16 || HOUT == 32, "map sizes of the three nets");
    static_assert(!(STRIDE == 1 && H == 32), "the 32x32 stride-1 layer lives in tcx_first.cuh");
};

struct XArgs {
    const __half* in;
    void* out;
    const __half* wpk;
    const float* bias;
    float inv_scale;
    int n, group;
    const int* count;
};

template <int CIN, int COUT, int H, int STRIDE, int NSPLIT, int STAGES, int OUT, int SA, int SW, int OSA>
struct XCfg {
    using In = XIn<H, STRIDE>;
    static constexpr int CO = COUT, STRD = STRIDE, OUTL = OUT, SPLIT_A = SA, SPLIT_W = SW, SPLIT_O = OSA;
    static constexpr int KC = CIN / 8, NT = COUT / NSPLIT, HOUT = In::HOUT;
    static constexpr int G = KC * (1 + SA);
    static constexpr int GS = STAGES * In::SLOT_STAGE + (STRIDE == 1 ? In::RW : 0);
    static constexpr int ACCW = 3 * NT;
    static constexpr int BLOCKS = 2 * In::TILES;
    static constexpr uint32_t W_BYTES = 9u * CIN * NT * 2u * (1 + SW);
    static constexpr uint32_t IN_BYTES = (uint32_t)G * GS * 16u;
    static constexpr uint32_t HI_IN_BYTES = (uint32_t)KC * In::NPLANES * In::DATA * 16u;
    static constexpr uint32_t UNIT_IN_BYTES = HI_IN_BYTES * (1 + SA);
    static constexpr int THREADS = 288;
    static constexpr size_t SMEM = 1024 + (size_t)W_BYTES + IN_BYTES;
    static constexpr size_t HI_OUT_BYTES = (size_t)(COUT / 8) * layout_slots(OUT) * 16;
    static constexpr size_t UNIT_OUT_BYTES = (OUT == L_HEAD) ? 0 : HI_OUT_BYTES * (1 + OSA);
    static constexpr int NR1 = (1 + SW) * 3 * NT;
    static constexpr int NRO = (1 + SW) * 2 * NT, NRE = (1 + SW) * NT;
    static_assert(CIN % 16 == 0 && NT % 16 == 0 && ACCW <= 256, "wgmma shape");
    static_assert(In::W == 8 || In::W == 16, "a warp's 16 accumulator rows hold whole image rows");
    static_assert(SA <= 1 && SW <= 1 && OSA <= 1, "split-precision switches are 0 | 1");
    static_assert(2 * STAGES + 1 <= 60, "barrier area");
    static_assert(SMEM <= 232448, "shared memory budget");
    static_assert(GS < 16384, "leading-byte offset field");
    static_assert(OUT == L_HEAD || layout_pair(OUT) || !In::PAIR, "a pair layer writes pair layouts or the head operand");
};

__device__ __forceinline__ float frag_left_even(float v1, int lane) { return __shfl_sync(0xffffffffu, v1, (lane + 28) & 31); }
__device__ __forceinline__ float frag_right_odd(float v0, int lane) { return __shfl_sync(0xffffffffu, v0, (lane + 4) & 31); }

__device__ __forceinline__ bool xpatch_valid(const XArgs& a, int pi) { return pi < a.n && (a.count == nullptr || (pi % a.group) < a.count[pi / a.group]); }

template <class Cfg, int BF>
__device__ __forceinline__ void xconv_block_issue(float* d, uint32_t a_t, uint32_t w_base) {
    using In = typename Cfg::In;
    constexpr int KC = Cfg::KC, NT = Cfg::NT, GS = Cfg::GS, RW = In::RW, SA = Cfg::SPLIT_A, SW = Cfg::SPLIT_W;
    constexpr uint32_t LBO_A = ((uint32_t)GS) << 16;
    wgmma_fence();
    if (Cfg::STRD == 1) {
#pragma unroll
        for (int dy = 0; dy < 3; dy++) {
#pragma unroll
            for (int j = 0; j < KC / 2; j++) {
                const uint32_t ahi = ((a_t + (uint32_t)(dy * RW + 2 * j * GS)) & 0x3FFFu) | LBO_A;
                const uint32_t alo = ((a_t + (uint32_t)(dy * RW + (KC + 2 * j) * GS)) & 0x3FFFu) | LBO_A;
                const uint32_t blk = w_base + (uint32_t)((dy * (KC / 2) + j) * 2 * Cfg::NR1);
                const uint32_t bhi = (blk & 0x3FFFu) | ((uint32_t)Cfg::NR1 << 16), blo = ((blk + 3 * NT) & 0x3FFFu) | ((uint32_t)Cfg::NR1 << 16);
                Wgmma<3 * NT, BF>::mma(d, desc64(ahi), desc64(bhi), (dy | j) != 0);
                if (SW) Wgmma<3 * NT, BF>::mma(d, desc64(ahi), desc64(blo), 1);
                if (SA) Wgmma<3 * NT, BF>::mma(d, desc64(alo), desc64(bhi), 1);
            }
        }
    } else {
#pragma unroll
        for (int dy = 0; dy < 3; dy++) {
            constexpr int PL = In::PLANE;
            const int py = (dy == 1) ? 0 : 1, ro = (dy == 0) ? 0 : 1;
#pragma unroll
            for (int j = 0; j < KC / 2; j++) {
                const uint32_t blk = w_base + (uint32_t)((dy * (KC / 2) + j) * 2 * (Cfg::NRO + Cfg::NRE));
                const uint32_t bo_hi = (blk & 0x3FFFu) | ((uint32_t)Cfg::NRO << 16), bo_lo = ((blk + 2 * NT) & 0x3FFFu) | ((uint32_t)Cfg::NRO << 16);
                const uint32_t be = blk + 2 * Cfg::NRO;
                const uint32_t be_hi = (be & 0x3FFFu) | ((uint32_t)Cfg::NRE << 16), be_lo = ((be + NT) & 0x3FFFu) | ((uint32_t)Cfg::NRE << 16);
                const uint32_t ao = a_t + (uint32_t)((py * 2 + 1) * PL + ro * RW);
                const uint32_t ao_hi = ((ao + (uint32_t)(2 * j * GS)) & 0x3FFFu) | LBO_A, ao_lo = ((ao + (uint32_t)((KC + 2 * j) * GS)) & 0x3FFFu) | LBO_A;
                Wgmma<2 * NT, BF>::mma(d, desc64(ao_hi), desc64(bo_hi), (dy | j) != 0);
                if (SW) Wgmma<2 * NT, BF>::mma(d, desc64(ao_hi), desc64(bo_lo), 1);
                if (SA) Wgmma<2 * NT, BF>::mma(d, desc64(ao_lo), desc64(bo_hi), 1);
                const uint32_t ae = a_t + (uint32_t)((py * 2 + 0) * PL + ro * RW);
                const uint32_t ae_hi = ((ae + (uint32_t)(2 * j * GS)) & 0x3FFFu) | LBO_A, ae_lo = ((ae + (uint32_t)((KC + 2 * j) * GS)) & 0x3FFFu) | LBO_A;
                Wgmma<NT, BF>::mma(d + NT, desc64(ae_hi), desc64(be_hi), (dy | j) != 0);
                if (SW) Wgmma<NT, BF>::mma(d + NT, desc64(ae_hi), desc64(be_lo), 1);
                if (SA) Wgmma<NT, BF>::mma(d + NT, desc64(ae_lo), desc64(be_hi), 1);
            }
        }
    }
    wgmma_commit();
}
template <class Cfg, int BF>
__device__ __forceinline__ void xconv_block_epilogue(const float* d, const XArgs& a, const float* s_bias, int u, int b, int split, int wq, int lane) {
    using In = typename Cfg::In;
    constexpr int NT = Cfg::NT, HOUT = Cfg::HOUT, W = In::W, PAIR = In::PAIR, COUT = Cfg::CO, OUT = Cfg::OUTL, OSA = Cfg::SPLIT_O;
    unsigned char* obase[2];
    bool ok[2];
    size_t lo_off = 0;
    const int i = lane >> 2, xi = PAIR ? (i & 3) : i;
    const bool has_l0 = xi > 0, has_r1 = xi < W / 2 - 1;
    static_assert(W == 16 || PAIR, "neighbour-paired row groups: 16 pixels, or 8 of each patch of a pair");
#pragma unroll
    for (int h = 0; h < 2; h++) {
        const int y = b * 4 + wq, x = 2 * xi + h, pi = PAIR ? 2 * u + (i >> 2) : u;
        ok[h] = xpatch_valid(a, pi);
        if (OUT == L_HEAD) {
            obase[h] = reinterpret_cast<unsigned char*>(a.out) + (((size_t)(pi >> 7) * (HOUT * HOUT * COUT / 8) + (size_t)(y * HOUT + x) * (COUT / 8)) * 128 + (pi & 127)) * 16;
            lo_off = (size_t)((a.n + 127) >> 7) * (HOUT * HOUT * COUT / 8) * 128 * 16;
        } else {
            const int ou = layout_pair(OUT) ? (pi >> 1) : pi;
            obase[h] = reinterpret_cast<unsigned char*>(a.out) + (size_t)ou * Cfg::UNIT_OUT_BYTES + (size_t)layout_slot(OUT, y, x, pi & 1) * 16;
            lo_off = (size_t)(COUT / 8) * layout_slots(OUT) * 16;
        }
    }
#pragma unroll
    for (int j = 0; j < NT / 8; j++) {
        const int c = j * 8 + 2 * (lane & 3);
        float v[2][2];
#pragma unroll
        for (int e = 0; e < 2; e++) {
            const float c00 = d[4 * j + e], c01 = d[4 * j + 2 + e];
            const float c10 = d[4 * (j + NT / 8) + e], c11 = d[4 * (j + NT / 8) + 2 + e];
            const float c20 = d[4 * (j + 2 * NT / 8) + e], c21 = d[4 * (j + 2 * NT / 8) + 2 + e];
            const float l0 = frag_left_even(c01, lane);
            float acc0, acc1;
            if (Cfg::STRD == 1) {
                const float r1 = frag_right_odd(c20, lane);
                const float t0 = c21 + c10, t1 = has_r1 ? r1 + c11 : c11;
                acc0 = has_l0 ? l0 + t0 : t0;
                acc1 = c00 + t1;
            } else {
                const float t0 = c10 + c20, t1 = c11 + c21;
                acc0 = has_l0 ? l0 + t0 : t0;
                acc1 = c00 + t1;
            }
            v[0][e] = fmaxf(fmaf(acc0, a.inv_scale, s_bias[c + e]), 0.f);
            v[1][e] = fmaxf(fmaf(acc1, a.inv_scale, s_bias[c + e]), 0.f);
        }
        const int ch = split * NT + c;
        const size_t goff = ((OUT == L_HEAD) ? (size_t)(ch / 8) * 128 * 16 : (size_t)(ch / 8) * layout_slots(OUT) * 16) + (ch & 7) * 2;
#pragma unroll
        for (int h = 0; h < 2; h++) {
            if (!ok[h]) continue;
            uint32_t hi, lo;
            split_pack2<OSA, BF>(v[h][0], v[h][1], hi, lo);
            *reinterpret_cast<uint32_t*>(obase[h] + goff) = hi;
            if (OSA) *reinterpret_cast<uint32_t*>(obase[h] + lo_off + goff) = lo;
        }
    }
}

template <int CIN, int COUT, int H, int STRIDE, int NSPLIT, int STAGES, int OUT, int SA, int SW, int OSA, int BF = 0, int MC = 0, int PPS = 0>
__global__ void __launch_bounds__(288, 1) tcx_conv_kernel(const XArgs a) {
    static_assert(MC == 0 || NSPLIT == 2, "multicast pairs the two channel-split CTAs");
    using Cfg = XCfg<CIN, COUT, H, STRIDE, NSPLIT, STAGES, OUT, SA, SW, OSA>;
    using In = typename Cfg::In;
    constexpr int ACCW = Cfg::ACCW, BLOCKS = Cfg::BLOCKS, GS = Cfg::GS, RW = In::RW;
    constexpr int PAIR = In::PAIR;
    constexpr bool PP = AG_CONV_PINGPONG && PPS;
    extern __shared__ __align__(1024) unsigned char smem[];
    uint64_t* full = reinterpret_cast<uint64_t*>(smem);
    uint64_t* empty = full + STAGES;
    uint64_t* wbar = empty + STAGES;
    float* s_bias = reinterpret_cast<float*>(smem + 512);
    unsigned char* sW = smem + 1024;
    unsigned char* sIn = sW + Cfg::W_BYTES;

    const int warp = threadIdx.x >> 5, lane = threadIdx.x & 31;
    const int split = blockIdx.y;
    const int n_units = PAIR ? (a.n + 1) >> 1 : a.n;

    int* s_tl_slot = reinterpret_cast<int*>(smem + 496);

    if (threadIdx.x < Cfg::NT) s_bias[threadIdx.x] = a.bias[split * Cfg::NT + threadIdx.x];
    if (threadIdx.x == 0) {
        for (int s = 0; s < STAGES; s++) { mbar_init(&full[s], 1); mbar_init(&empty[s], (PP ? 8 : 2) * (1 + MC)); }
        mbar_init(wbar, 1);
        asm volatile("fence.mbarrier_init.release.cluster;" ::: "memory");
    }
    ConvTimeline::claim(s_tl_slot);
    for (int i = threadIdx.x; i < (int)(Cfg::IN_BYTES / 16); i += blockDim.x) reinterpret_cast<uint4*>(sIn)[i] = make_uint4(0, 0, 0, 0);
    asm volatile("fence.proxy.async.shared::cta;" ::: "memory");
    __syncthreads();
    if (MC) cluster_sync();
    ConvTimeline tl;
    tl.init(s_tl_slot);
    auto release = [&](uint64_t* e) {
        if (MC) { mbar_arrive_cluster(e, 0); mbar_arrive_cluster(e, 1); }
        else mbar_arrive(e);
    };

    auto uvalid = [&](int u) -> bool { return PAIR ? (xpatch_valid(a, 2 * u) || xpatch_valid(a, 2 * u + 1)) : xpatch_valid(a, u); };

    if (warp == 8) {
        if (lane == 0) {
            mbar_expect_tx(wbar, Cfg::W_BYTES);
            bulk_g2s(sW, reinterpret_cast<const unsigned char*>(a.wpk) + (size_t)split * Cfg::W_BYTES, Cfg::W_BYTES, wbar);
            int it = 0;
            for (int u = blockIdx.x; u < n_units; u += gridDim.x) {
                if (!uvalid(u)) continue;
                const int s = it % STAGES;
                tl.lap(CT_OTHER);
                mbar_wait(&empty[s], ((it / STAGES) & 1) ^ 1);
                tl.lap(CT_WAIT_EMPTY);
                mbar_expect_tx(&full[s], Cfg::UNIT_IN_BYTES);
                const unsigned char* gsrc = reinterpret_cast<const unsigned char*>(a.in) + (size_t)u * Cfg::UNIT_IN_BYTES;
#pragma unroll 1
                for (int g = 0; g < Cfg::G; g++)
#pragma unroll
                    for (int pl = 0; pl < In::NPLANES; pl++) {
                        unsigned char* dst = sIn + ((size_t)g * GS + (size_t)s * In::SLOT_STAGE + (size_t)pl * In::PLANE + RW) * 16;
                        const unsigned char* srcp = gsrc + ((size_t)g * In::NPLANES + pl) * In::DATA * 16;
                        if (MC) { if (((g * In::NPLANES + pl) & 1) == split) bulk_g2s_mc(dst, srcp, In::DATA * 16u, &full[s], (uint16_t)3); }
                        else bulk_g2s(dst, srcp, In::DATA * 16u, &full[s]);
                    }
                it++;
            }
            tl.lap(CT_OTHER);
            if (MC) {
                for (int k = 0; k < STAGES && k < it; k++) { const int j = it - 1 - k; mbar_wait(&empty[j % STAGES], (j / STAGES) & 1); }
            }
            tl.lap(CT_WAIT_EMPTY);
        }
    } else if (warp < 8) {
        const int wg = warp >> 2, wq = warp & 3;
        mbar_wait(wbar, 0);
        const uint32_t w_base = smem_u32(sW) >> 4;
        const uint32_t in_base = smem_u32(sIn) >> 4;
        int it = 0;
        for (int u = blockIdx.x; u < n_units; u += gridDim.x) {
            if (!uvalid(u)) continue;
            const int s = it % STAGES;
            tl.lap(CT_OTHER);
            mbar_wait(&full[s], (it / STAGES) & 1);
            tl.lap(CT_WAIT_FULL);
            const uint32_t st_base = in_base + (uint32_t)(s * In::SLOT_STAGE);
#pragma unroll 1
            for (int b = wg; b < BLOCKS; b += 2) {
                float d[ACCW / 2];
                if (PP && (wg == 1 || it > 0 || b > 0)) bar_sync(XORDER + wg, 256);
                tl.lap(CT_TURN);
                tl.event(0);
                xconv_block_issue<Cfg, BF>(d, st_base + (uint32_t)(b * 64), w_base);
                if (PP) asm volatile("bar.arrive %0, 256;" ::"r"(XORDER + (wg ^ 1)) : "memory");
                tl.lap(CT_ISSUE);
                wgmma_wait<0>();
                wgmma_reg_fence<ACCW / 2>(d);
                tl.lap(CT_MMA_WAIT);
                tl.event(1);
                if (PP && b + 2 >= BLOCKS && lane == 0) release(&empty[s]);
                xconv_block_epilogue<Cfg, BF>(d, a, s_bias, u, b, split, wq, lane);
                tl.lap(CT_EPILOGUE);
                tl.event(2);
            }
            if (!PP) {
                bar_sync(3 + wg, 128);
                tl.lap(CT_WG_BAR);
                if ((threadIdx.x & 127) == 0) release(&empty[s]);
            }
            it++;
        }
        if (PP && wg == 0 && it > 0) bar_sync(XORDER, 256);
        tl.lap(CT_OTHER);
    }
    tl.finish();
    __syncthreads();
    if (MC) cluster_sync();
}

}
}
```

### include/affnet_b200.h

```cpp
#ifndef AFFNET_B200_H
#define AFFNET_B200_H

#include <stddef.h>
#include <stdint.h>

#ifdef __cplusplus
extern "C" {
#endif

#define AG_OK 0
#define AG_ERR_INVALID -1
#define AG_ERR_CUDA -2
#define AG_ERR_CAPACITY -3
#define AG_ERR_NO_DEVICE -4

#define AG_MAX_OCTAVES 16
#define AG_MAX_LEVELS 8

const char* ag_last_error(void);
int ag_abi_version(void);

int ag_prof_begin(void* stream);
int ag_prof_end(void);
int ag_prof_get(int i, const char** name, float* ms);

typedef struct {
    int B, H, W;
    int n_octaves;
    int n_levels;
    int h[AG_MAX_OCTAVES], w[AG_MAX_OCTAVES];
    long long level_offset[AG_MAX_OCTAVES][AG_MAX_LEVELS];
    long long total_floats;
    double sigma[AG_MAX_OCTAVES][AG_MAX_LEVELS];
    double blur_sigma[AG_MAX_OCTAVES][AG_MAX_LEVELS];
    double pix_dist[AG_MAX_OCTAVES];
} ag_pyramid_plan_t;

int ag_pyramid_plan(int B, int H, int W, int nlevels, double init_sigma, int border, ag_pyramid_plan_t* plan);

int ag_pyramid_build(const ag_pyramid_plan_t* plan, const float* d_img, float* d_pyr, void* stream);

int ag_gaussian_blur(const float* d_in, float* d_out, int B, int h, int w, double sigma, void* stream);

int ag_hessian_response(const float* d_in, float* d_out, int B, int h, int w, double sigma, float th, void* stream);

typedef struct {
    int B;
    int cand_cap;
    int n_level_slots;
    float* d_cand_val;
    uint32_t* d_cand_seq;
    float* d_cand_scyx;
    float* d_cand_aux;
    int* d_cand_count;
    int* d_level_pos;
    int* d_level_emit;
    int* d_variants;
    uint8_t* d_octave_maps;
} ag_detect_ws_t;

size_t ag_detect_ws_bytes(const ag_pyramid_plan_t* plan, int cand_cap);
int ag_detect_ws_carve(const ag_pyramid_plan_t* plan, int cand_cap, void* d_ws, ag_detect_ws_t* ws);

int ag_detect(const ag_pyramid_plan_t* plan, const float* d_pyr, float th, int mr_border, ag_detect_ws_t* ws, void* stream);

int ag_detect_level_from_responses(const float* d_low, const float* d_cur, const float* d_high, int h, int w,
                                   const double scales[3], int mr_border, const uint8_t* d_omap_in,
                                   uint8_t* d_omap_out, int slot, ag_detect_ws_t* ws, void* stream);

int ag_select_keypoints(const ag_pyramid_plan_t* plan, const ag_detect_ws_t* ws, int num_features, float a_scale,
                        int out_cap, float* d_resp, float* d_lafs, int* d_oct, int* d_lvl, int* d_count,
                        void* stream);

size_t ag_select_all_workspace_bytes(const ag_pyramid_plan_t* plan, int cand_cap);
int ag_select_all_keypoints(const ag_pyramid_plan_t* plan, const ag_detect_ws_t* ws, float a_scale, int out_cap,
                            void* d_scratch, size_t scratch_bytes, float* d_resp, float* d_lafs, int* d_oct, int* d_lvl,
                            int* d_count, void* stream);

int ag_extract_patches(const float* d_img, int C, int h, int w, int per_patch_img, const float* d_lafs, int n,
                       int PS, float* d_out, void* stream);

int ag_extract_patches_pyr(const ag_pyramid_plan_t* plan, const float* d_pyr, const float* d_lafs, const int* d_oct,
                           const int* d_lvl, const int* d_count, int cap, int PS, float* d_out, void* stream);

int ag_pyramid_level_for_lafs(const ag_pyramid_plan_t* plan, const float* d_dlafs, int n, int PS, int* d_oct,
                              int* d_lvl, void* stream);

#define AG_NET_AFFNET 0
#define AG_NET_ORINET 1
#define AG_NET_HARDNET 2

typedef struct ag_net ag_net_t;

int ag_net_create(int kind, const float* h_blob, size_t n_floats, ag_net_t** out);
void ag_net_destroy(ag_net_t* net);
size_t ag_net_blob_floats(int kind);
int ag_net_set_engine(ag_net_t* net, int engine);
int ag_net_get_engine(const ag_net_t* net);
int ag_debug_pyramid_mode(int fused);
int ag_debug_tcx_layer(const ag_net_t* net, const float* d_patches, int n, int upto, float* d_out, void* d_ws, size_t ws_bytes, void* stream);
int ag_debug_libm(const float* d_y, const float* d_x, int n, float* d_atan2, float* d_cos, float* d_sin, void* stream);
int ag_debug_orientation_hist_pyr(const ag_pyramid_plan_t* plan, const float* d_pyr, const float* d_lafs, const int* d_oct, const int* d_lvl,
                                  const int* d_count, int cap, int PS, const float* h_gk, float* d_R, void* stream);
int ag_debug_baumberg_pyr(const ag_pyramid_plan_t* plan, const float* d_pyr, const float* d_lafs, const int* d_oct, const int* d_lvl,
                          const int* d_count, int cap, int PS, int iters, const float* h_gk, float* d_A, void* stream);
size_t ag_net_workspace_bytes(int kind, int n);

int ag_affnet_forward(const ag_net_t* net, const float* d_patches, int n, const int* d_count, int group, float* d_out,
                      void* d_ws, size_t ws_bytes, void* stream);
int ag_orinet_forward(const ag_net_t* net, const float* d_patches, int n, const int* d_count, int group, float* d_out,
                      float* d_angle, void* d_ws, size_t ws_bytes, void* stream);
int ag_hardnet_forward(const ag_net_t* net, const float* d_patches, int n, const int* d_count, int group, float* d_out,
                       void* d_ws, size_t ws_bytes, void* stream);

int ag_affnet_forward_raw(const ag_net_t* net, const float* d_patches, int n, float* d_raw, void* d_ws, size_t ws_bytes, void* stream);
int ag_orinet_forward_raw(const ag_net_t* net, const float* d_patches, int n, float* d_raw, void* d_ws, size_t ws_bytes, void* stream);
int ag_net_forward_pyr(const ag_net_t* net, const ag_pyramid_plan_t* plan, const float* d_pyr, const float* d_lafs, const int* d_oct,
                       const int* d_lvl, const int* d_count, int cap, float* d_out, void* d_ws, size_t ws_bytes, void* stream);

int ag_affine_shape_filter(const float* d_A, const float* d_resp, const float* d_lafs, const int* d_oct,
                           const int* d_lvl, const int* d_count_in, int B, int cap, int num_features, int out_cap,
                           float* d_resp_out, float* d_lafs_out, int* d_oct_out, int* d_lvl_out, int* d_count_out,
                           void* stream);
int ag_affine_shape_filter_all(const float* d_A, const float* d_resp, const float* d_lafs, const int* d_oct, const int* d_lvl,
                               const int* d_count_in, int B, int cap, float* d_resp_out, float* d_lafs_out, int* d_oct_out,
                               int* d_lvl_out, int* d_count_out, void* stream);

int ag_lafs_apply_rotation(float* d_lafs, const float* d_R, int n, void* stream);
int ag_lafs_scale(const float* d_in, float* d_out, int n, float a_coef, float x_coef, float y_coef, void* stream);
int ag_mat2_compose(const float* d_A, const float* d_B, float* d_out, int n, void* stream);
int ag_lafs_left_multiply(const float* d_A, const float* d_lafs, float* d_out, int n, void* stream);
int ag_lafs_to_ell(const float* d_lafs, int n, float* d_ell, void* stream);

int ag_circular_gauss_kernel(int kernlen, double sigma, float* h_out);
int ag_orientation_hist(const float* d_patches, int n, int PS, const float* d_gk, float* d_angle, void* stream);
int ag_baumberg_shape(const float* d_patches, int n, int PS, const float* d_gk, float* d_A, void* stream);

int ag_sift_windows(int PS, float* h_gk, float* h_pk, int* k, int* stride);
int ag_sift_describe(const float* d_patches, int n, int PS, float clipval, float* d_out, void* stream);
int ag_sift_describe_pyr(const ag_pyramid_plan_t* plan, const float* d_pyr, const float* d_lafs, const int* d_oct, const int* d_lvl,
                         const int* d_count, int cap, int PS, float clipval, float* d_out, void* stream);

int ag_distance_matrix(const float* d_a, int n1, const float* d_b, int n2, int dim, float* d_out, void* stream);
size_t ag_match_snn_workspace_bytes(int n1, int n2);
int ag_match_snn(const float* d_desc1, int n1, const float* d_desc2, int n2, int dim, float ratio, void* d_ws, size_t ws_bytes, int* d_idx2,
                 float* d_min, float* d_second, unsigned char* d_keep, void* stream);

size_t ag_match_pairs_workspace_bytes(int S1, int cap1, int S2, int cap2, int P);
int ag_match_pairs(const float* d_desc1, const int* d_count1, int S1, int cap1, const float* d_desc2, const int* d_count2, int S2, int cap2,
                   int dim, const int* d_pairs, int P, float ratio, void* d_ws, size_t ws_bytes, int* d_idx2, float* d_min, float* d_second,
                   unsigned char* d_keep, int* d_tent, int* d_ntent, void* stream);

int ag_homography_ransac(const float* d_lafs1, int S1, int cap1, const float* d_lafs2, int S2, int cap2, const int* d_pairs, int P,
                         const int* d_tent, const int* d_ntent, int tcap, float inl_th, float confidence, int max_iters, unsigned long long seed,
                         float* d_H, unsigned char* d_inl, int* d_ninl, int* d_iters, void* stream);
int ag_gt_correspondences_pairs(const float* d_lafs1, int S1, int cap1, const float* d_lafs2, int S2, int cap2, const int* d_pairs, int P,
                                const int* d_tent, const int* d_ntent, int tcap, const float* d_H1to2, float dist_threshold,
                                float* d_min_dist, int* d_idx2, int* d_true, int* d_ntrue, void* stream);

typedef struct ag_pipeline ag_pipeline_t;

typedef struct {
    int B, H, W;
    int num_features;
    int nlevels;
    int border;
    double init_sigma;
    double mrSize;
    int do_ori;
    int cand_cap;
} ag_pipeline_config_t;

int ag_pipeline_create(const ag_pipeline_config_t* cfg, const ag_net_t* affnet, const ag_net_t* orinet,
                       const ag_net_t* hardnet, ag_pipeline_t** out);

#define AG_SHAPE_NONE 0
#define AG_SHAPE_AFFNET 1
#define AG_SHAPE_BAUMBERG 2
#define AG_ORI_NONE 0
#define AG_ORI_ORINET 1
#define AG_ORI_HISTOGRAM 2
typedef struct {
    int shape;
    int num_baum_iters;
    int shape_ps;
    int ori;
    int ori_ps;
} ag_pipeline_estimators_t;
int ag_pipeline_create_ex(const ag_pipeline_config_t* cfg, const ag_pipeline_estimators_t* est, const ag_net_t* affnet,
                          const ag_net_t* orinet, const ag_net_t* hardnet, ag_pipeline_t** out);

#define AG_DESC_HARDNET 0
#define AG_DESC_SIFT 1
typedef struct {
    int kind;
    int ps;
    float clipval;
} ag_pipeline_descriptor_t;
int ag_pipeline_create_desc(const ag_pipeline_config_t* cfg, const ag_pipeline_estimators_t* est, const ag_pipeline_descriptor_t* desc,
                            const ag_net_t* affnet, const ag_net_t* orinet, const ag_net_t* hardnet, ag_pipeline_t** out);
int ag_pipeline_create_th(const ag_pipeline_config_t* cfg, const ag_pipeline_estimators_t* est, const ag_pipeline_descriptor_t* desc,
                          float th, const ag_net_t* affnet, const ag_net_t* orinet, const ag_net_t* hardnet, ag_pipeline_t** out);
void ag_pipeline_destroy(ag_pipeline_t* p);
size_t ag_pipeline_workspace_bytes(const ag_pipeline_t* p);
const ag_pyramid_plan_t* ag_pipeline_plan(const ag_pipeline_t* p);
int ag_pipeline_run(ag_pipeline_t* p, const float* d_img, void* d_ws, size_t ws_bytes, float* d_lafs, float* d_resp,
                    float* d_desc, int* d_count, void* stream);
int ag_pipeline_launch_count(const ag_pipeline_t* p);

#ifdef __cplusplus
}
#endif
#endif
```

Before: 681.1.

## Fuse AffNet linear head into last conv layer epilogue via mma.sync

```diff
diff --git a/affnet_b200/_lib.py b/affnet_b200/_lib.py
--- a/affnet_b200/_lib.py
+++ b/affnet_b200/_lib.py
@@ -92,6 +92,7 @@
     "ag_orinet_forward_raw": (i32, [vp, vp, i32, vp, vp, sz, vp]),
     "ag_debug_pyramid_mode": (i32, [i32]),
     "ag_debug_tcx_layer": (i32, [vp, vp, i32, i32, vp, vp, sz, vp]),
+    "ag_debug_affnet_unfused_raw": (i32, [vp, vp, i32, vp, vp, sz, vp]),
     "ag_debug_libm": (i32, [vp, vp, i32, vp, vp, vp, vp]),
     "ag_debug_orientation_hist_pyr": (i32, [C.POINTER(PyramidPlan), vp, vp, vp, vp, vp, i32, i32, vp, vp, vp]),
     "ag_debug_baumberg_pyr": (i32, [C.POINTER(PyramidPlan), vp, vp, vp, vp, vp, i32, i32, i32, vp, vp, vp]),
diff --git a/affnet_b200/csrc/net_impl.cuh b/affnet_b200/csrc/net_impl.cuh
--- a/affnet_b200/csrc/net_impl.cuh
+++ b/affnet_b200/csrc/net_impl.cuh
@@ -11,6 +11,10 @@
 #define AG_ENGINE_TC2 4
 #define AG_ENGINE_TC2_BF16 5
 #define AG_ENGINE_TC_FAST 3
+
+#ifndef AG_FUSED_HEAD
+#define AG_FUSED_HEAD 1
+#endif
 
 struct ag_net {
     int kind;
@@ -26,6 +30,7 @@
     __half* d_headh;
     float* d_head_w;
     float* d_head_b;
+    const uint32_t* d_head_wt;
     float* d_head_bx;
     float w_inv_scale[6];
     float head_inv_scale;
@@ -54,8 +59,14 @@
 int tcx_split_w(int kind, int layer);
 int tcx_stride(int layer);
 size_t tcx_act_bytes(int n);
+struct FusedHead {
+    float* out;
+    float* raw;
+};
+bool tcx_head_fused(const ag_net* net);
+void tcx_head_aff_weights(const float* hw, float scale, std::vector<__half>& out);
 int tcx_trunk_affori(const ag_net* net, const tc::FirstSrc& src, int n, int group, const int* count, void* bufA, void* bufB, void* feat,
-                     cudaStream_t st, int upto);
+                     cudaStream_t st, int upto, const FusedHead* fh = nullptr);
 int tcx_trunk_hardnet(const ag_net* net, const tc::FirstSrc& src, int n, int group, const int* count, void* bufA, void* bufB, void* headbuf,
                       cudaStream_t st, int upto, int bf16 = 0);
 int tc_hardnet_head(const ag_net* net, const void* headbuf, int n, int group, const int* count, float* out, cudaStream_t st, int bf16 = 0);
diff --git a/affnet_b200/csrc/nets_simt.cu b/affnet_b200/csrc/nets_simt.cu
--- a/affnet_b200/csrc/nets_simt.cu
+++ b/affnet_b200/csrc/nets_simt.cu
@@ -439,6 +439,12 @@
                         dst[(chunk * 64 + 32 + o) * 8 + e] = __float2half_rn(v - __half2float(hi));
                     }
     }
+    size_t hwt_off = 0;
+    if (kind == AG_NET_AFFNET) {
+        while (packed_h.size() % 8) packed_h.push_back(__float2half_rn(0.f));
+        hwt_off = packed_h.size();
+        tcx_head_aff_weights(packed.data() + hw_off, head_scale, packed_h);
+    }
     ag_net* net = new ag_net();
     memset(net, 0, sizeof(*net));
     net->kind = kind;
@@ -475,6 +481,7 @@
     net->d_head_w = net->d_all + hw_off;
     net->d_head_b = net->d_all + hb_off;
     net->d_head_bx = net->d_all + hbx_off;
+    net->d_head_wt = kind == AG_NET_AFFNET ? reinterpret_cast<const uint32_t*>(net->d_all_h + hwt_off) : nullptr;
     *out = net;
     return AG_OK;
 }
@@ -539,7 +546,7 @@
 }
 
 static int run_trunk(const ag_net* net, const float* patches, const tc::FirstSrc* pyr_src, int n, int group, const int* count, float* a,
-                     float* b, float** feat, cudaStream_t st) {
+                     float* b, float** feat, cudaStream_t st, const FusedHead* fh = nullptr) {
     if (net->engine != AG_ENGINE_SIMT) {
         const tc::FirstSrc src = pyr_src ? *pyr_src : tc_src_patches(patches);
         char* base = (char*)a;
@@ -553,7 +560,7 @@
         b = (float*)(base + 2 * act);
         *feat = b;
         if (net->kind == AG_NET_HARDNET) { set_error("HardNet tensor-core path has its own entry"); return AG_ERR_INVALID; }
-        if (net->engine == AG_ENGINE_TC2) return tcx_trunk_affori(net, src, n, group, count, bufA, bufB, b, st, 6);
+        if (net->engine == AG_ENGINE_TC2) return tcx_trunk_affori(net, src, n, group, count, bufA, bufB, b, st, 6, fh);
         if (net->engine != AG_ENGINE_TC_FAST) return tc_trunk_orinet(net, src, n, group, count, bufA, bufB, b, st);
         return tc_trunk_affnet(net, src, n, group, count, bufA, bufB, b, st);
     }
@@ -579,7 +586,7 @@
 extern "C" {
 
 static int affnet_impl(const ag_net_t* net, const float* d_patches, const tc::FirstSrc* src, int n, const int* d_count, int group,
-                       float* d_out, void* d_ws, size_t ws_bytes, void* stream, float* d_raw = nullptr) {
+                       float* d_out, void* d_ws, size_t ws_bytes, void* stream, float* d_raw = nullptr, bool unfused = false) {
     AG_REQUIRE(net && (d_patches || src) && (d_out || d_raw), "NULL argument");
     AG_REQUIRE(net->kind == AG_NET_AFFNET, "not an AffNet handle");
     if (n <= 0) return AG_OK;
@@ -588,6 +595,10 @@
     int rc = split_ws(net->kind, n, d_ws, ws_bytes, &a, &b);
     if (rc) return rc;
     cudaStream_t st = (cudaStream_t)stream;
+    if (tcx_head_fused(net) && !unfused) {
+        const FusedHead fh = {d_out, d_raw};
+        return run_trunk(net, d_patches, src, n, group, d_count, a, b, &b, st, &fh);
+    }
     if ((rc = run_trunk(net, d_patches, src, n, group, d_count, a, b, &b, st))) return rc;
     if (net->engine == AG_ENGINE_TC || net->engine == AG_ENGINE_TC_FAST || net->engine == AG_ENGINE_TC2) return tc_headx_forward(net, b, n, group, d_count, d_out, nullptr, st, d_raw);
     AG_REQUIRE(d_raw == nullptr && d_out, "raw head outputs need a tensor-core engine with the GEMM head (1, 3 or 4)");
@@ -658,6 +669,10 @@
     AG_REQUIRE(d_patches && d_raw, "NULL argument");
     return affnet_impl(net, d_patches, nullptr, n, nullptr, n, nullptr, d_ws, ws_bytes, stream, d_raw);
 }
+int ag_debug_affnet_unfused_raw(const ag_net_t* net, const float* d_patches, int n, float* d_raw, void* d_ws, size_t ws_bytes, void* stream) {
+    AG_REQUIRE(d_patches && d_raw, "NULL argument");
+    return affnet_impl(net, d_patches, nullptr, n, nullptr, n, nullptr, d_ws, ws_bytes, stream, d_raw, true);
+}
 int ag_orinet_forward_raw(const ag_net_t* net, const float* d_patches, int n, float* d_raw, void* d_ws, size_t ws_bytes, void* stream) {
     AG_REQUIRE(d_patches && d_raw, "NULL argument");
     return orinet_impl(net, d_patches, nullptr, n, nullptr, n, nullptr, nullptr, d_ws, ws_bytes, stream, d_raw);
diff --git a/affnet_b200/csrc/nets_tcx.cu b/affnet_b200/csrc/nets_tcx.cu
--- a/affnet_b200/csrc/nets_tcx.cu
+++ b/affnet_b200/csrc/nets_tcx.cu
@@ -34,13 +34,14 @@
 }
 
 template <int CIN, int COUT, int H, int STRIDE, int NSPLIT, int STAGES, int OUT, int SA, int SW, int OSA, int BF = 0, int MC = 0, int PPS = 0>
-static int launch_conv(const void* in, void* out, const __half* w, const float* b, float inv_scale, int n, int group, const int* count, cudaStream_t st) {
+static int launch_conv(const void* in, void* out, const __half* w, const float* b, float inv_scale, int n, int group, const int* count, cudaStream_t st,
+                       const XArgs* head = nullptr) {
     using Cfg = XCfg<CIN, COUT, H, STRIDE, NSPLIT, STAGES, OUT, SA, SW, OSA>;
     auto kern = tcx_conv_kernel<CIN, COUT, H, STRIDE, NSPLIT, STAGES, OUT, SA, SW, OSA, BF, MC, PPS>;
     static bool configured[64] = {};
     int rc = ensure_smem_attr((const void*)kern, (int)Cfg::SMEM, configured, "tcx_conv smem attr");
     if (rc != AG_OK) return rc;
-    XArgs a;
+    XArgs a = head ? *head : XArgs{};
     a.in = (const __half*)in; a.out = out; a.wpk = w; a.bias = b; a.inv_scale = inv_scale; a.n = n; a.group = group; a.count = count;
     const int units = Cfg::In::PAIR ? (n + 1) / 2 : n;
     int gx = num_sms() / NSPLIT;
@@ -70,7 +71,7 @@
     static bool configured[64] = {};
     int rc = ensure_smem_attr((const void*)kern, (int)Cfg::SMEM, configured, "tcx_first smem attr");
     if (rc != AG_OK) return rc;
-    XArgs a;
+    XArgs a = {};
     a.in = nullptr; a.out = out; a.wpk = w; a.bias = b; a.inv_scale = inv_scale; a.n = n; a.group = group; a.count = count;
     XArgs a3 = a;
     a3.out = out3; a3.wpk = w3; a3.bias = b3; a3.inv_scale = inv_scale3;
@@ -173,7 +174,7 @@
 #define AG_HARD_MC6 0
 #endif
 int tcx_trunk_affori(const ag_net* net, const tc::FirstSrc& src0, int n, int group, const int* count, void* bufA, void* bufB, void* feat,
-                     cudaStream_t st, int upto) {
+                     cudaStream_t st, int upto, const FusedHead* fh) {
     using namespace tcx;
     tc::FirstSrc src = src0;
     src.w1 = net->d_w1; src.b1 = net->d_b[0]; src.w1_inv = net->w_inv_scale[0]; src.w1_scale = 1.0f / net->w_inv_scale[0];
@@ -186,7 +187,34 @@
     if (upto <= 4) return AG_OK;
     if ((rc = launch_conv<32, 64, 16, 2, 1, 2, L_S1_8P, 1, 1, 1>(bufB, bufA, net->d_wx[4], net->d_b[4], net->w_inv_scale[4], n, group, count, st))) return rc;
     if (upto <= 5) return AG_OK;
+    if (fh) {
+        if (!tcx_head_fused(net)) { set_error("the fused head exists for AffNet's second-generation engine"); return AG_ERR_INVALID; }
+        XArgs h = {};
+        h.hw = net->d_head_wt; h.hinv = net->head_inv_scale; h.hb = net->d_head_b; h.hout = fh->out; h.hraw = fh->raw;
+        return launch_conv<64, 64, 8, 1, 1, 2, L_HEAD_AFF, 1, 1, 1, 0, 0, 1>(bufA, nullptr, net->d_wx[5], net->d_b[5], net->w_inv_scale[5], n, group, count, st, &h);
+    }
     return launch_conv<64, 64, 8, 1, 1, 2, L_HEAD, 1, 1, 1, 0, 0, 1>(bufA, feat, net->d_wx[5], net->d_b[5], net->w_inv_scale[5], n, group, count, st);
+}
+
+bool tcx_head_fused(const ag_net* net) { return AG_FUSED_HEAD && net->kind == AG_NET_AFFNET && net->engine == AG_ENGINE_TC2; }
+
+void tcx_head_aff_weights(const float* hw, float scale, std::vector<__half>& out) {
+    using namespace tcx;
+    const size_t base = out.size();
+    out.resize(base + (size_t)HEAD_AFF_W * 256 * 2);
+    for (int t = 0; t < 256; t++) {
+        const int g = t >> 7, wq = (t >> 5) & 3, lane = t & 31, y = 4 * g + wq, x = lane >> 2;
+        for (int o = 0; o < 3; o++)
+            for (int jj = 0; jj < 4; jj++)
+                for (int part = 0; part < 2; part++)
+                    for (int r = 0; r < 2; r++)
+                        for (int e = 0; e < 2; e++) {
+                            const int c = 16 * jj + 2 * (lane & 3) + 8 * r + e;
+                            const float v = scale * hw[(size_t)o * 4096 + c * 64 + y * 8 + x];
+                            const __half hi = __float2half_rn(v);
+                            out[base + ((size_t)head_aff_idx(o, jj, part, r) * 256 + t) * 2 + e] = part == 0 ? hi : __float2half_rn(v - __half2float(hi));
+                        }
+    }
 }
 
 template <int BF>
diff --git a/affnet_b200/csrc/tcx_conv.cuh b/affnet_b200/csrc/tcx_conv.cuh
--- a/affnet_b200/csrc/tcx_conv.cuh
+++ b/affnet_b200/csrc/tcx_conv.cuh
@@ -13,6 +13,7 @@
 using namespace ag::tc;
 
 constexpr int XORDER = 5;
+constexpr int XHEAD = 7;
 
 enum { CT_TOTAL, CT_WAIT_FULL, CT_TURN, CT_ISSUE, CT_MMA_WAIT, CT_EPILOGUE, CT_WG_BAR, CT_WAIT_EMPTY, CT_OTHER, CT_STATES };
 #ifdef AG_CONV_TIMELINE
@@ -54,7 +55,7 @@
 };
 #endif
 
-enum XLayout { L_S2_16 = 0, L_S1_16 = 1, L_S2_8P = 2, L_S1_8P = 3, L_HEAD = 4 };
+enum XLayout { L_S2_16 = 0, L_S1_16 = 1, L_S2_8P = 2, L_S1_8P = 3, L_HEAD = 4, L_HEAD_AFF = 5 };
 
 __device__ __forceinline__ void bulk_g2s_mc(void* dst, const void* src, uint32_t bytes, uint64_t* bar, uint16_t mask) {
     asm volatile("cp.async.bulk.shared::cluster.global.mbarrier::complete_tx::bytes.multicast::cluster [%0], [%1], %2, [%3], %4;" ::"r"(smem_u32(dst)),
@@ -139,6 +140,11 @@
     float inv_scale;
     int n, group;
     const int* count;
+    const uint32_t* hw;
+    float hinv;
+    const float* hb;
+    float* hout;
+    float* hraw;
 };
 
 template <int CIN, int COUT, int H, int STRIDE, int NSPLIT, int STAGES, int OUT, int SA, int SW, int OSA>
@@ -155,9 +161,11 @@
     static constexpr uint32_t HI_IN_BYTES = (uint32_t)KC * In::NPLANES * In::DATA * 16u;
     static constexpr uint32_t UNIT_IN_BYTES = HI_IN_BYTES * (1 + SA);
     static constexpr int THREADS = 288;
-    static constexpr size_t SMEM = 1024 + (size_t)W_BYTES + IN_BYTES;
+    static constexpr bool FUSED_HEAD = OUT == L_HEAD_AFF;
+    static constexpr uint32_t HEAD_BYTES = FUSED_HEAD ? 2u * 64u * 2u * 3u * 2u * 4u : 0u;
+    static constexpr size_t SMEM = 1024 + (size_t)W_BYTES + IN_BYTES + HEAD_BYTES;
     static constexpr size_t HI_OUT_BYTES = (size_t)(COUT / 8) * layout_slots(OUT) * 16;
-    static constexpr size_t UNIT_OUT_BYTES = (OUT == L_HEAD) ? 0 : HI_OUT_BYTES * (1 + OSA);
+    static constexpr size_t UNIT_OUT_BYTES = (OUT >= L_HEAD) ? 0 : HI_OUT_BYTES * (1 + OSA);
     static constexpr int NR1 = (1 + SW) * 3 * NT;
     static constexpr int NRO = (1 + SW) * 2 * NT, NRE = (1 + SW) * NT;
     static_assert(CIN % 16 == 0 && NT % 16 == 0 && ACCW <= 256, "wgmma shape");
@@ -166,7 +174,8 @@
     static_assert(2 * STAGES + 1 <= 60, "barrier area");
     static_assert(SMEM <= 232448, "shared memory budget");
     static_assert(GS < 16384, "leading-byte offset field");
-    static_assert(OUT == L_HEAD || layout_pair(OUT) || !In::PAIR, "a pair layer writes pair layouts or the head operand");
+    static_assert(OUT >= L_HEAD || layout_pair(OUT) || !In::PAIR, "a pair layer writes pair layouts or the head operand");
+    static_assert(!FUSED_HEAD || (CIN == 64 && COUT == 64 && H == 8 && STRIDE == 1 && NSPLIT == 1), "the fused head is AffNet's layer 6");
 };
 
 __device__ __forceinline__ float frag_left_even(float v1, int lane) { return __shfl_sync(0xffffffffu, v1, (lane + 28) & 31); }
@@ -220,6 +229,32 @@
     }
     wgmma_commit();
 }
+template <class Cfg>
+__device__ __forceinline__ void xconv_frag_values(const float* d, const XArgs& a, const float* s_bias, int j, int lane, bool has_l0, bool has_r1, float (&v)[2][2]) {
+    constexpr int NT = Cfg::NT;
+    const int c = j * 8 + 2 * (lane & 3);
+#pragma unroll
+    for (int e = 0; e < 2; e++) {
+        const float c00 = d[4 * j + e], c01 = d[4 * j + 2 + e];
+        const float c10 = d[4 * (j + NT / 8) + e], c11 = d[4 * (j + NT / 8) + 2 + e];
+        const float c20 = d[4 * (j + 2 * NT / 8) + e], c21 = d[4 * (j + 2 * NT / 8) + 2 + e];
+        const float l0 = frag_left_even(c01, lane);
+        float acc0, acc1;
+        if (Cfg::STRD == 1) {
+            const float r1 = frag_right_odd(c20, lane);
+            const float t0 = c21 + c10, t1 = has_r1 ? r1 + c11 : c11;
+            acc0 = has_l0 ? l0 + t0 : t0;
+            acc1 = c00 + t1;
+        } else {
+            const float t0 = c10 + c20, t1 = c11 + c21;
+            acc0 = has_l0 ? l0 + t0 : t0;
+            acc1 = c00 + t1;
+        }
+        v[0][e] = fmaxf(fmaf(acc0, a.inv_scale, s_bias[c + e]), 0.f);
+        v[1][e] = fmaxf(fmaf(acc1, a.inv_scale, s_bias[c + e]), 0.f);
+    }
+}
+
 template <class Cfg, int BF>
 __device__ __forceinline__ void xconv_block_epilogue(const float* d, const XArgs& a, const float* s_bias, int u, int b, int split, int wq, int lane) {
     using In = typename Cfg::In;
@@ -247,26 +282,7 @@
     for (int j = 0; j < NT / 8; j++) {
         const int c = j * 8 + 2 * (lane & 3);
         float v[2][2];
-#pragma unroll
-        for (int e = 0; e < 2; e++) {
-            const float c00 = d[4 * j + e], c01 = d[4 * j + 2 + e];
-            const float c10 = d[4 * (j + NT / 8) + e], c11 = d[4 * (j + NT / 8) + 2 + e];
-            const float c20 = d[4 * (j + 2 * NT / 8) + e], c21 = d[4 * (j + 2 * NT / 8) + 2 + e];
-            const float l0 = frag_left_even(c01, lane);
-            float acc0, acc1;
-            if (Cfg::STRD == 1) {
-                const float r1 = frag_right_odd(c20, lane);
-                const float t0 = c21 + c10, t1 = has_r1 ? r1 + c11 : c11;
-                acc0 = has_l0 ? l0 + t0 : t0;
-                acc1 = c00 + t1;
-            } else {
-                const float t0 = c10 + c20, t1 = c11 + c21;
-                acc0 = has_l0 ? l0 + t0 : t0;
-                acc1 = c00 + t1;
-            }
-            v[0][e] = fmaxf(fmaf(acc0, a.inv_scale, s_bias[c + e]), 0.f);
-            v[1][e] = fmaxf(fmaf(acc1, a.inv_scale, s_bias[c + e]), 0.f);
-        }
+        xconv_frag_values<Cfg>(d, a, s_bias, j, lane, has_l0, has_r1, v);
         const int ch = split * NT + c;
         const size_t goff = ((OUT == L_HEAD) ? (size_t)(ch / 8) * 128 * 16 : (size_t)(ch / 8) * layout_slots(OUT) * 16) + (ch & 7) * 2;
 #pragma unroll
@@ -278,6 +294,73 @@
             if (OSA) *reinterpret_cast<uint32_t*>(obase[h] + lo_off + goff) = lo;
         }
     }
+}
+
+__host__ __device__ constexpr int head_aff_idx(int o, int jj, int part, int r) { return ((o * 4 + jj) * 2 + part) * 2 + r; }
+constexpr int HEAD_AFF_W = 48;
+constexpr int HEAD_AFF_STAGE = 64 * 2 * 3 * 2;
+
+__device__ __forceinline__ void mma16816(float (&c)[4], const uint32_t (&a)[4], uint32_t b0, uint32_t b1, bool acc) {
+    const float z = 0.f;
+    asm volatile("mma.sync.aligned.m16n8k16.row.col.f32.f16.f16.f32 {%0,%1,%2,%3}, {%4,%5,%6,%7}, {%8,%9}, {%10,%11,%12,%13};"
+                 : "=f"(c[0]), "=f"(c[1]), "=f"(c[2]), "=f"(c[3])
+                 : "r"(a[0]), "r"(a[1]), "r"(a[2]), "r"(a[3]), "r"(b0), "r"(b1), "f"(acc ? c[0] : z), "f"(acc ? c[1] : z), "f"(acc ? c[2] : z),
+                   "f"(acc ? c[3] : z));
+}
+
+template <class Cfg>
+__device__ __forceinline__ void xconv_block_head(const float* d, const XArgs& a, const float* s_bias, const uint32_t (&hb)[HEAD_AFF_W], int lane, int y, float* s_stage) {
+    const int i = lane >> 2, xi = i & 3, p = lane >> 4;
+    const bool has_l0 = xi > 0, has_r1 = xi < 3;
+    float ch[3][4], cl[3][4];
+#pragma unroll
+    for (int jj = 0; jj < 4; jj++) {
+        uint32_t ah[4], al[4];
+#pragma unroll
+        for (int half = 0; half < 2; half++) {
+            float v[2][2];
+            xconv_frag_values<Cfg>(d, a, s_bias, 2 * jj + half, lane, has_l0, has_r1, v);
+#pragma unroll
+            for (int h = 0; h < 2; h++) split_pack2<1, 0>(v[h][0], v[h][1], ah[2 * half + h], al[2 * half + h]);
+        }
+#pragma unroll
+        for (int o = 0; o < 3; o++) {
+            mma16816(ch[o], ah, hb[head_aff_idx(o, jj, 0, 0)], hb[head_aff_idx(o, jj, 0, 1)], jj > 0);
+            mma16816(ch[o], al, hb[head_aff_idx(o, jj, 0, 0)], hb[head_aff_idx(o, jj, 0, 1)], true);
+            mma16816(cl[o], ah, hb[head_aff_idx(o, jj, 1, 0)], hb[head_aff_idx(o, jj, 1, 1)], jj > 0);
+        }
+    }
+    if ((lane & 3) == xi) {
+#pragma unroll
+        for (int h = 0; h < 2; h++) {
+            float* q = s_stage + ((y * 8 + 2 * xi + h) * 2 + p) * 6;
+#pragma unroll
+            for (int o = 0; o < 3; o++) { q[2 * o] = ch[o][3 * h]; q[2 * o + 1] = cl[o][3 * h]; }
+        }
+    }
+}
+
+__device__ __forceinline__ void head_aff_tail(const XArgs& a, const float* st, int u, int lane) {
+    float acc = 0.f;
+    if (lane < 6) {
+        const int p = lane / 3, o = lane % 3;
+        float th = 0.f, tl = 0.f;
+#pragma unroll 8
+        for (int k = 0; k < 64; k++) {
+            th += st[(k * 2 + p) * 6 + 2 * o];
+            tl += st[(k * 2 + p) * 6 + 2 * o + 1];
+        }
+        acc = th + tl;
+    }
+    const int base = lane < 3 ? 0 : 3;
+    const float s0 = __shfl_sync(0xffffffffu, acc, base) * a.hinv, s1 = __shfl_sync(0xffffffffu, acc, base + 1) * a.hinv,
+                s2 = __shfl_sync(0xffffffffu, acc, base + 2) * a.hinv;
+    if (lane != 0 && lane != 3) return;
+    const int pi = 2 * u + lane / 3;
+    if (!xpatch_valid(a, pi)) return;
+    const float a00 = 1.0f + tanhf(s0 + a.hb[0]), a10 = tanhf(s1 + a.hb[1]), a11 = 1.0f + tanhf(s2 + a.hb[2]);
+    if (a.hraw) { a.hraw[(size_t)pi * 3] = a00; a.hraw[(size_t)pi * 3 + 1] = a10; a.hraw[(size_t)pi * 3 + 2] = a11; }
+    if (a.hout) rectify_up_is_up(a00, 0.f, a10, a11, a.hout + (size_t)pi * 4);
 }
 
 template <int CIN, int COUT, int H, int STRIDE, int NSPLIT, int STAGES, int OUT, int SA, int SW, int OSA, int BF = 0, int MC = 0, int PPS = 0>
@@ -295,6 +378,8 @@
     float* s_bias = reinterpret_cast<float*>(smem + 512);
     unsigned char* sW = smem + 1024;
     unsigned char* sIn = sW + Cfg::W_BYTES;
+    float* s_head = reinterpret_cast<float*>(sIn + Cfg::IN_BYTES);
+    static_assert(!Cfg::FUSED_HEAD || BLOCKS == 2, "fused head: warpgroup g takes block g of every unit");
 
     const int warp = threadIdx.x >> 5, lane = threadIdx.x & 31;
     const int split = blockIdx.y;
@@ -354,6 +439,11 @@
         }
     } else if (warp < 8) {
         const int wg = warp >> 2, wq = warp & 3;
+        uint32_t hw[Cfg::FUSED_HEAD ? HEAD_AFF_W : 1];
+        if constexpr (Cfg::FUSED_HEAD) {
+#pragma unroll
+            for (int k = 0; k < HEAD_AFF_W; k++) hw[k] = __ldg(a.hw + k * 256 + threadIdx.x);
+        }
         mbar_wait(wbar, 0);
         const uint32_t w_base = smem_u32(sW) >> 4;
         const uint32_t in_base = smem_u32(sIn) >> 4;
@@ -379,9 +469,18 @@
                 tl.lap(CT_MMA_WAIT);
                 tl.event(1);
                 if (PP && b + 2 >= BLOCKS && lane == 0) release(&empty[s]);
-                xconv_block_epilogue<Cfg, BF>(d, a, s_bias, u, b, split, wq, lane);
+                if constexpr (Cfg::FUSED_HEAD) xconv_block_head<Cfg>(d, a, s_bias, hw, lane, 4 * wg + wq, s_head + (it & 1) * HEAD_AFF_STAGE);
+                else xconv_block_epilogue<Cfg, BF>(d, a, s_bias, u, b, split, wq, lane);
                 tl.lap(CT_EPILOGUE);
                 tl.event(2);
+            }
+            if constexpr (Cfg::FUSED_HEAD) {
+                const int hbar = XHEAD + (it & 1);
+                if (wg == 0) asm volatile("bar.arrive %0, 256;" ::"r"(hbar) : "memory");
+                else {
+                    bar_sync(hbar, 256);
+                    if (wq == 0) head_aff_tail(a, s_head + (it & 1) * HEAD_AFF_STAGE, u, lane);
+                }
             }
             if (!PP) {
                 bar_sync(3 + wg, 128);
diff --git a/include/affnet_b200.h b/include/affnet_b200.h
--- a/include/affnet_b200.h
+++ b/include/affnet_b200.h
@@ -99,6 +99,7 @@
 int ag_net_get_engine(const ag_net_t* net);
 int ag_debug_pyramid_mode(int fused);
 int ag_debug_tcx_layer(const ag_net_t* net, const float* d_patches, int n, int upto, float* d_out, void* d_ws, size_t ws_bytes, void* stream);
+int ag_debug_affnet_unfused_raw(const ag_net_t* net, const float* d_patches, int n, float* d_raw, void* d_ws, size_t ws_bytes, void* stream);
 int ag_debug_libm(const float* d_y, const float* d_x, int n, float* d_atan2, float* d_cos, float* d_sin, void* stream);
 int ag_debug_orientation_hist_pyr(const ag_pyramid_plan_t* plan, const float* d_pyr, const float* d_lafs, const int* d_oct, const int* d_lvl,
                                   const int* d_count, int cap, int PS, const float* h_gk, float* d_R, void* stream);
```

Result: faster. 690.3, median of 6 (+1.3%).
